# treangenlab/komb

Hardware: AMD Instinct MI355X
Metric: peeled edges/sec (k-truss) (higher is better)
Workload: dtype int32

## Files before the change

komb_amd/api.py:

```python
import ctypes
import os

import numpy as np

from . import _lib
from ._lib import KombOpts, KombStats, as_c, ptr


class KombError(RuntimeError):
    def __init__(self, code, msg):
        super().__init__(f"komb_accel error {code}: {msg}")
        self.code = code


def gen_hug_edges(nv, n_cliques, alpha=2.6, seed=42):
    lib = _lib.load()
    n_raw = lib.komb_gen_hug_edges(nv, n_cliques, alpha, seed, None)
    if n_raw < 0:
        raise ValueError("komb_gen_hug_edges: bad arguments")
    uv = np.empty((n_raw, 2), dtype=np.int64)
    got = lib.komb_gen_hug_edges(nv, n_cliques, alpha, seed, ptr(uv))
    assert got == n_raw
    return uv


FORWARD_ENV_OPTIONS = False
OPTION_NAMES = ("FINISH", "LOCAL_LIMIT", "LOCAL_ITEMS", "LOCAL_DENSITY", "LOCAL_DEFER_CHUNKS", "TAIL", "CORE_TAIL", "INDEX",
                "REC_CAP", "OWN_DENSE_CAP", "NO_OWN_DENSE", "NO_REC_SCRATCH", "NO_FIRST_QUEUE", "FULL_CAPS", "PREP_ROW_STAGE", "RETIRE_EVERY", "SHARD_ENGINE",
                "TRI_DEBUG", "POOL_DEBUG", "BUILD_DEBUG", "LOCAL_DEBUG", "TAIL_DEBUG", "COMP_SAMPLE", "COMM_SHORT", "COMM_HEAVY", "POISON")

SENTINEL_I32 = -0x5A5A5A5B


def _out_i32(n):
    return np.full(n, SENTINEL_I32, dtype=np.int32)


def _out_f64(n):
    return np.full(n, np.nan, dtype=np.float64)


class KombAccel:
    def __init__(self, device=0, verbosity=0, flags=0):
        self._lib = _lib.load()
        opts = KombOpts(device=device, verbosity=verbosity)
        opts.reserved[0] = flags
        self._ctx = self._lib.komb_create(ctypes.byref(opts))
        if not self._ctx:
            raise MemoryError("komb_create failed")
        self.device = device
        self.nv = -1
        self.ne = 0
        self._forwarded = {}

    def set_option(self, name, value):
        v = None if value is None else str(value).encode()
        self._check(self._lib.komb_set_option(self._ctx, name.encode(), v))

    def _sync_env_options(self):
        if not FORWARD_ENV_OPTIONS:
            return
        for name in OPTION_NAMES:
            v = os.environ.get("KOMB_" + name)
            if name == "INDEX" and os.environ.get("KOMB_TWO_PASS"):
                v = "two_pass"
            if name == "SHARD_ENGINE" and v is None:
                v = os.environ.get("KOMB_SHARD_PEEL")
            if self._forwarded.get(name) != v:
                self.set_option(name, v)
                self._forwarded[name] = v

    def close(self):
        if getattr(self, "_ctx", None):
            self._lib.komb_destroy(self._ctx)
            self._ctx = None

    def __del__(self):
        self.close()

    def __enter__(self):
        return self

    def __exit__(self, *a):
        self.close()

    def _check(self, rc):
        if rc != 0:
            raise KombError(rc, self._lib.komb_last_error(self._ctx).decode())

    def from_edges(self, nv, uv):
        uv = as_c(np.asarray(uv).reshape(-1, 2), np.int64)
        self._sync_env_options()
        self._check(self._lib.komb_graph_from_edges(self._ctx, nv, uv.shape[0], ptr(uv)))
        self._info()
        return self

    def from_csr(self, rowptr, col):
        rowptr = as_c(rowptr, np.int64)
        col = as_c(col, np.int32)
        self._sync_env_options()
        self._check(self._lib.komb_graph_from_csr(self._ctx, len(rowptr) - 1, ptr(rowptr), ptr(col)))
        self._info()
        return self

    def _info(self):
        nv, ne = ctypes.c_int64(), ctypes.c_int64()
        self._check(self._lib.komb_graph_info(self._ctx, ctypes.byref(nv), ctypes.byref(ne)))
        self.nv, self.ne = nv.value, ne.value

    def get_csr(self):
        rowptr = np.full(self.nv + 1, SENTINEL_I32, dtype=np.int64)
        col = _out_i32(2 * self.ne)
        self._check(self._lib.komb_graph_get_csr(self._ctx, ptr(rowptr), ptr(col)))
        return rowptr, col

    def core_run(self):
        self._sync_env_options()
        self._check(self._lib.komb_core_run(self._ctx))

    def set_shard_peel(self, on=True):
        self._check(self._lib.komb_set_shard_peel(self._ctx, 1 if on else 0))

    def core_fetch(self):
        deg = _out_i32(self.nv)
        core = _out_i32(self.nv)
        self._check(self._lib.komb_core_fetch(self._ctx, ptr(deg), ptr(core)))
        return deg, core

    def run_core(self):
        self.core_run()
        return self.core_fetch()

    def onion_run(self):
        self._sync_env_options()
        self._check(self._lib.komb_onion_run(self._ctx))

    def onion_fetch(self):
        layer = _out_i32(self.nv)
        core = _out_i32(self.nv)
        self._check(self._lib.komb_onion_fetch(self._ctx, ptr(layer), ptr(core)))
        return layer, core

    def run_onion(self):
        self.onion_run()
        return self.onion_fetch()

    def onion_info(self):
        n, k, ms = ctypes.c_int64(), ctypes.c_int32(), ctypes.c_double()
        self._check(self._lib.komb_onion_info(self._ctx, ctypes.byref(n), ctypes.byref(k), ctypes.byref(ms)))
        return {"n_layers": n.value, "max_coreness": k.value, "ms": ms.value}

    COMP_KINDS = {"core": _lib.KOMB_COMP_CORE, "truss": _lib.KOMB_COMP_TRUSS}

    def components_run(self, kind, k):
        self._sync_env_options()
        self._check(self._lib.komb_components_run(self._ctx, self.COMP_KINDS.get(kind, kind), k))

    def components_fetch(self):
        label = _out_i32(max(self.nv, 0))
        size = _out_i32(max(self.nv, 0))
        self._check(self._lib.komb_components_fetch(self._ctx, ptr(label), ptr(size)))
        return label, size

    def components_info(self):
        kind, k = ctypes.c_int32(), ctypes.c_int32()
        mem, comp, big, ms = ctypes.c_int64(), ctypes.c_int64(), ctypes.c_int64(), ctypes.c_double()
        self._check(self._lib.komb_components_info(self._ctx, ctypes.byref(kind), ctypes.byref(k), ctypes.byref(mem),
                                                   ctypes.byref(comp), ctypes.byref(big), ctypes.byref(ms)))
        return {"kind": kind.value, "k_used": k.value, "n_members": mem.value, "n_components": comp.value,
                "largest": big.value, "ms": ms.value}

    def run_components(self, kind="core", k=0):
        self.components_run(kind, k)
        return self.components_fetch()

    def truss_run(self, vmask=None):
        if vmask is not None:
            vmask = as_c(vmask, np.uint8)
            if len(vmask) != self.nv:
                raise ValueError("vmask must have nv entries")
        self._sync_env_options()
        self._check(self._lib.komb_truss_run(self._ctx, ptr(vmask)))

    def truss_run_slice(self, rank, world, vmask=None):
        if vmask is not None:
            vmask = as_c(vmask, np.uint8)
            if len(vmask) != self.nv:
                raise ValueError("vmask must have nv entries")
        self._sync_env_options()
        self._check(self._lib.komb_truss_run_slice(self._ctx, ptr(vmask), int(rank), int(world)))

    def truss_prepare(self):
        self._check(self._lib.komb_truss_prepare(self._ctx))

    def truss_unprepare(self):
        self._check(self._lib.komb_truss_unprepare(self._ctx))

    def graph_moments(self):
        self._check(self._lib.komb_graph_moments(self._ctx))

    def truss_fetch_into(self, eu=None, ev=None, tr=None):
        self._check(self._lib.komb_truss_fetch(self._ctx, ptr(eu) if eu is not None else None, ptr(ev) if ev is not None else None,
                                               ptr(tr) if tr is not None else None))

    def truss_fetch(self, with_support=False):
        n = ctypes.c_int64()
        self._check(self._lib.komb_truss_count(self._ctx, ctypes.byref(n)))
        eu = _out_i32(n.value)
        ev = _out_i32(n.value)
        tr = _out_i32(n.value)
        self._check(self._lib.komb_truss_fetch(self._ctx, ptr(eu), ptr(ev), ptr(tr)))
        if not with_support:
            return eu, ev, tr
        sup = _out_i32(n.value)
        self._check(self._lib.komb_truss_fetch_support(self._ctx, ptr(sup)))
        return eu, ev, tr, sup

    def run_truss(self, vmask=None, with_support=False):
        self.truss_run(vmask)
        return self.truss_fetch(with_support)

    def truss_communities_run(self, k=3):
        self._sync_env_options()
        self._check(self._lib.komb_truss_communities_run(self._ctx, k))

    def truss_communities_fetch(self):
        n = ctypes.c_int64()
        self._check(self._lib.komb_truss_count(self._ctx, ctypes.byref(n)))
        label = _out_i32(max(n.value, 0))
        size = _out_i32(max(n.value, 0))
        self._check(self._lib.komb_truss_communities_fetch(self._ctx, ptr(label), ptr(size)))
        return label, size

    def truss_communities_fetch_vertices(self):
        n_comm = _out_i32(max(self.nv, 0))
        self._check(self._lib.komb_truss_communities_fetch_vertices(self._ctx, ptr(n_comm)))
        return n_comm

    def truss_communities_info(self):
        k = ctypes.c_int32()
        mem, comm, big, multi, ms = ctypes.c_int64(), ctypes.c_int64(), ctypes.c_int64(), ctypes.c_int64(), ctypes.c_double()
        self._check(self._lib.komb_truss_communities_info(self._ctx, ctypes.byref(k), ctypes.byref(mem), ctypes.byref(comm),
                                                          ctypes.byref(big), ctypes.byref(multi), ctypes.byref(ms)))
        return {"k_used": k.value, "n_member_edges": mem.value, "n_communities": comm.value, "largest": big.value,
                "n_multi_vertices": multi.value, "ms": ms.value}

    def run_truss_communities(self, k=3):
        self.truss_communities_run(k)
        return self.truss_communities_fetch()

    def get_anomaly_score(self, degree, coreness):
        degree = as_c(degree, np.int32)
        coreness = as_c(coreness, np.int32)
        score = _out_f64(len(degree))
        self._sync_env_options()
        self._check(self._lib.komb_corea_scores(self._ctx, ptr(degree), ptr(coreness), len(degree), ptr(score)))
        return score

    def fractional_ranks(self, degree, coreness):
        degree = as_c(degree, np.int32)
        coreness = as_c(coreness, np.int32)
        rd = _out_f64(len(degree))
        rk = _out_f64(len(degree))
        self._sync_env_options()
        self._check(self._lib.komb_corea_ranks(self._ctx, ptr(degree), ptr(coreness), len(degree), ptr(rd), ptr(rk)))
        return rd, rk

    def densest_block(self, suspiciousness=None):
        n = int(self.nv)
        order = _out_i32(max(2 * n, 1))
        side = _out_i32(max(2 * n, 1))
        self._sync_env_options()
        nb = ctypes.c_int64(0)
        dens = ctypes.c_double(0.0)
        susp = None if suspiciousness is None else as_c(suspiciousness, np.float64)
        self._check(self._lib.komb_densest_block(self._ctx, ptr(susp), ptr(order), ptr(side), ctypes.byref(nb), ctypes.byref(dens)))
        return order[: 2 * n], side[: 2 * n], int(nb.value), float(dens.value)

    def stats(self):
        st = KombStats()
        self._check(self._lib.komb_get_stats(self._ctx, ctypes.byref(st)))
        return {name: getattr(st, name) for name, _ in KombStats._fields_}
```

komb_amd/csrc/common.h:

```cpp
#pragma once

#include <hip/hip_runtime.h>

#include <chrono>
#include <cstddef>
#include <cstdint>
#include <cstdio>
#include <cstdlib>
#include <cstring>
#include <map>
#include <string>
#include <vector>

#include "komb_accel.h"

#include <roctracer/roctx.h>

namespace komb {

struct Range {
    explicit Range(const char *name) { (void)roctxRangePushA(name); }
    ~Range() { (void)roctxRangePop(); }
    void next(const char *name) { (void)roctxRangePop(); (void)roctxRangePushA(name); }
    Range(const Range &) = delete;
    Range &operator=(const Range &) = delete;
};

constexpr int kBlock = 256;
constexpr int kWave = 64;
constexpr int32_t kAlive = 0x7FFFFFFF;
constexpr int32_t kAliveMin = 0x40000000;

struct PeelCtrl {
    int32_t  mode;
    int32_t  level;
    int32_t  round;
    int32_t  done;
    uint32_t cur_light;
    uint32_t cur_heavy;
    int32_t  cur_sel;
    uint32_t remaining;
    int32_t  n_levels;
    int32_t  n_rounds;
    int32_t  n_scans;
    int32_t  max_level;
    uint32_t live_count;
    int32_t  live_sel;
    int32_t  live_mode;
    int32_t  seq;
    uint32_t tail_l[2];
    uint32_t tail_h[2];
    int32_t  next_min;
    uint32_t live_tail;
    int32_t  last_retire;
    uint32_t tail_limit;
    uint32_t pad1[7];
    int32_t  max_retire_gap;
};
static_assert(offsetof(PeelCtrl, seq) == 60 && offsetof(PeelCtrl, tail_l) == 64, "PeelCtrl: the entry state is one 64-byte line");
static_assert(sizeof(PeelCtrl) == 128, "PeelCtrl layout");

struct LocalCtrl {
    int32_t  done;
    int32_t  iters;
    uint32_t spare[3];
    uint32_t bad;
    int32_t  max_val;
    uint32_t levels;
    uint32_t evals;
    uint32_t n_light, n_heavy;
    uint32_t n_giant;
    uint32_t n_chunk;
    uint32_t pad0;
    unsigned long long key_sum;
};
static_assert(sizeof(LocalCtrl) == 64, "LocalCtrl layout");

enum FinishMode : int { FIN_LOCAL = 0, FIN_LDS = 1, FIN_NONE = 2 };

struct Timer {
    hipEvent_t a = nullptr, b = nullptr;
    bool init() { return hipEventCreate(&a) == hipSuccess && hipEventCreate(&b) == hipSuccess; }
    void start(hipStream_t s) { (void)hipEventRecord(a, s); }
    double stop(hipStream_t s)
    {
        (void)hipEventRecord(b, s);
        (void)hipEventSynchronize(b);
        float ms = 0.f;
        (void)hipEventElapsedTime(&ms, a, b);
        return (double)ms;
    }
    void destroy() { if (a) (void)hipEventDestroy(a); if (b) (void)hipEventDestroy(b); a = b = nullptr; }
};

struct EventSet {
    std::vector<hipEvent_t> v;
    EventSet() = default;
    EventSet(const EventSet &) = delete;
    EventSet &operator=(const EventSet &) = delete;
    hipError_t make(hipEvent_t *out, unsigned flags = 0)
    {
        hipEvent_t e = nullptr;
        const hipError_t rc = flags ? hipEventCreateWithFlags(&e, flags) : hipEventCreate(&e);
        if (rc == hipSuccess) { v.push_back(e); *out = e; }
        return rc;
    }
    ~EventSet() { for (hipEvent_t e : v) if (e) (void)hipEventDestroy(e); }
};

}

struct Poison {
    bool on = false;
    uint32_t word = 0;
    hipStream_t stream = nullptr;
    hipError_t fill(void *p, size_t bytes) const
    {
        if (!on || !p || !bytes) return hipSuccess;
        const size_t words = bytes / 4, rest = bytes % 4;
        hipError_t e = hipSuccess;
        if (words) e = hipMemsetD32Async((hipDeviceptr_t)p, (int)word, words, stream);
        if (e == hipSuccess && rest) e = hipMemsetAsync((char *)p + 4 * words, (int)(word & 0xFFu), rest, stream);
        return e == hipSuccess ? hipStreamSynchronize(stream) : e;
    }
    hipError_t malloc(void **out, size_t bytes) const
    {
        void *q = nullptr;
        hipError_t e = hipMalloc(&q, bytes);
        if (e != hipSuccess) return e;
        e = fill(q, bytes);
        if (e != hipSuccess) { (void)hipFree(q); return e; }
        *out = q;
        return hipSuccess;
    }
};

struct DevPool {
    struct Block { void *p; size_t bytes; bool used; };
    std::vector<Block> blocks;
    size_t n_malloc = 0, n_trim = 0;
    double ms_malloc = 0.0;
    Poison poison;
    hipError_t get(void **out, size_t bytes)
    {
        if (bytes == 0) bytes = 16;
        int best = -1;
        for (int i = 0; i < (int)blocks.size(); ++i)
            if (!blocks[i].used && blocks[i].bytes >= bytes && blocks[i].bytes <= bytes + bytes / 4 + 4096 &&
                (best < 0 || blocks[i].bytes < blocks[best].bytes)) best = i;
        if (best >= 0) {
            if (poison.on) { const hipError_t e = poison.fill(blocks[best].p, blocks[best].bytes); if (e != hipSuccess) return e; }
            blocks[best].used = true; *out = blocks[best].p; return hipSuccess;
        }
        void *q = nullptr;
        ++n_malloc;
        const auto t0 = std::chrono::steady_clock::now();
        hipError_t e = hipMalloc(&q, bytes);
        ms_malloc += std::chrono::duration<double, std::milli>(std::chrono::steady_clock::now() - t0).count();
        if (e != hipSuccess) {
            ++n_trim;
            trim();
            e = hipMalloc(&q, bytes);
            if (e != hipSuccess) return e;
        }
        blocks.push_back({q, bytes, true});
        if (poison.on) { e = poison.fill(q, bytes); if (e != hipSuccess) { put(q); return e; } }
        *out = q;
        return hipSuccess;
    }
    void put(void *p)
    {
        if (!p) return;
        for (auto &b : blocks) if (b.p == p) { b.used = false; return; }
    }
    size_t unused_bytes() const
    {
        size_t t = 0;
        for (const auto &b : blocks) if (!b.used) t += b.bytes;
        return t;
    }
    void trim()
    {
        std::vector<Block> keep;
        for (auto &b : blocks) { if (b.used) keep.push_back(b); else (void)hipFree(b.p); }
        blocks.swap(keep);
    }
    void clear()
    {
        for (auto &b : blocks) (void)hipFree(b.p);
        blocks.clear();
    }
};

struct TrussPrep {
    bool valid = false;
    int64_t nv = 0, ne = 0;
    int32_t  *o2i = nullptr, *i2o = nullptr;
    uint32_t *orow = nullptr;
    int32_t  *ocol = nullptr, *osrc = nullptr;
    uint32_t *e2k = nullptr;
    uint4    *vline = nullptr;
    void     *wtasks = nullptr;
    int64_t   n_wtasks = 0;
    int64_t   own_bound = 0;
    double    ms = 0.0;
    double    ms_part[4] = {0, 0, 0, 0};
};

struct komb_ctx {
    komb_opts opts{};
    DevPool pool;
    std::string err;
    bool device_ok = false;
    int device = 0;
    hipStream_t stream = nullptr;
    bool own_stream = false;
    komb::Timer timer;
    std::map<std::string, std::string> options;

    int64_t nv = -1, ne = 0;
    uint32_t *d_o_rowptr = nullptr;
    int32_t  *d_o_col = nullptr;
    TrussPrep prep;

    int32_t *d_deg = nullptr;
    int32_t *d_core = nullptr;
    bool core_done = false;

    int32_t *d_onion_layer = nullptr;
    int32_t *d_onion_core = nullptr;
    int64_t onion_layers = 0;
    int32_t onion_max_core = 0;
    double onion_ms = 0.0;
    bool onion_done = false;

    int32_t *d_comp_label = nullptr;
    int32_t *d_comp_size = nullptr;
    int32_t comp_kind = 0, comp_k = 0;
    int64_t comp_members = 0, comp_count = 0, comp_largest = 0;
    double comp_ms = 0.0;
    bool comp_done = false;

    int32_t *d_comm_label = nullptr;
    int32_t *d_comm_size = nullptr;
    int32_t *d_comm_ncomm = nullptr;
    int32_t comm_k = 0;
    int64_t comm_members = 0, comm_count = 0, comm_largest = 0, comm_multi = 0;
    double comm_ms = 0.0, comm_ms_vertices = 0.0;
    bool comm_done = false, comm_v_ready = false;

    int64_t t_ne = -1;
    int32_t *d_t_eu = nullptr, *d_t_ev = nullptr, *d_t_truss = nullptr, *d_t_sup = nullptr;
    uint2 *d_t_slice = nullptr;
    uint32_t t_k_lo = 0, t_k_hi = 0;
    bool t_sup_ready = false;
    bool t_own_edges = false;
    int32_t *d_ceu = nullptr, *d_cev = nullptr;
    bool truss_done = false;
    int slice_rank = 0, slice_world = 1;
    bool shard_peel = false;
    struct { int64_t nv = -1, m = -1; unsigned long long own_cap = 0, rec_cap = 0; } cap_hint;

    komb::PeelCtrl *h_ctrl = nullptr;
    komb::LocalCtrl *h_local = nullptr;
    void *h_stage = nullptr;
    struct H2DStager *stager = nullptr;

    komb_stats stats{};
};

inline hipError_t dev_malloc(komb_ctx *ctx, void **out, size_t bytes) { return ctx->pool.poison.malloc(out, bytes); }

inline const char *ctx_opt(const komb_ctx *ctx, const char *name)
{
    const auto it = ctx->options.find(name);
    return it == ctx->options.end() ? nullptr : it->second.c_str();
}
inline bool ctx_flag(const komb_ctx *ctx, const char *name)
{
    const char *v = ctx_opt(ctx, name);
    return v && strcmp(v, "0") != 0;
}
namespace komb {
inline FinishMode finish_mode(const komb_ctx *ctx, FinishMode dflt)
{
    const char *e = ctx_opt(ctx, "FINISH");
    if (e && !strcmp(e, "local")) return FIN_LOCAL;
    if (e && !strcmp(e, "lds")) return FIN_LDS;
    if (e && !strcmp(e, "none")) return FIN_NONE;
    return dflt;
}
inline uint64_t local_item_limit(const komb_ctx *ctx, uint64_t dflt)
{
    if (const char *e = ctx_opt(ctx, "LOCAL_ITEMS")) return strtoull(e, nullptr, 10);
    return dflt;
}
inline uint32_t local_density_limit(const komb_ctx *ctx, uint32_t dflt)
{
    if (const char *e = ctx_opt(ctx, "LOCAL_DENSITY")) return (uint32_t)strtoul(e, nullptr, 10);
    return dflt;
}
inline uint32_t local_limit(const komb_ctx *ctx, uint64_t units, uint64_t divisor)
{
    uint64_t l = units / divisor;
    if (l < 4096) l = 4096;
    if (const char *e = ctx_opt(ctx, "LOCAL_LIMIT")) l = strtoull(e, nullptr, 10);
    if (l > units) l = units;
    return (uint32_t)l;
}
}

struct DevBufs {
    komb_ctx *ctx;
    std::vector<void *> owned;
    explicit DevBufs(komb_ctx *c) : ctx(c) {}
    DevBufs(const DevBufs &) = delete;
    DevBufs &operator=(const DevBufs &) = delete;
    template <class T> hipError_t alloc(T **out, size_t count)
    {
        void *q = nullptr;
        hipError_t e = ctx->pool.get(&q, (count ? count : 1) * sizeof(T));
        if (e == hipSuccess) { owned.push_back(q); *out = (T *)q; }
        return e;
    }
    void detach(void *q)
    {
        for (auto &p : owned) if (p == q) p = nullptr;
    }
    void release(void *q)
    {
        for (auto &p : owned) if (p == q && q) { ctx->pool.put(q); p = nullptr; }
    }
    ~DevBufs() { for (void *p : owned) if (p) ctx->pool.put(p); }
};

#define KOMB_FAIL(ctx, code, ...)                                   \
    do {                                                            \
        char _b[512];                                               \
        snprintf(_b, sizeof(_b), __VA_ARGS__);                      \
        (ctx)->err = _b;                                            \
        return (code);                                              \
    } while (0)

#define KOMB_HIP(ctx, call)                                                          \
    do {                                                                             \
        hipError_t _e = (call);                                                      \
        if (_e != hipSuccess) {                                                      \
            hipError_t _nomem = hipErrorOutOfMemory;                                 \
            KOMB_FAIL(ctx, _e == _nomem ? KOMB_ERR_NOMEM : KOMB_ERR_DEVICE,          \
                      "%s failed: %s (%s:%d)", #call, hipGetErrorString(_e),         \
                      __FILE__, __LINE__);                                           \
        }                                                                            \
    } while (0)

#define KOMB_TRY(expr)                         \
    do {                                       \
        int _s = (expr);                       \
        if (_s != KOMB_OK) return _s;          \
    } while (0)

constexpr size_t kStageBytes = 64 << 10;
inline hipError_t d2h(komb_ctx *ctx, void *dst, const void *src, size_t bytes)
{
    if (ctx->h_stage && bytes <= kStageBytes && dst != ctx->h_stage) {
        hipError_t e = hipMemcpyAsync(ctx->h_stage, src, bytes, hipMemcpyDeviceToHost, ctx->stream);
        if (e == hipSuccess) e = hipStreamSynchronize(ctx->stream);
        if (e == hipSuccess) memcpy(dst, ctx->h_stage, bytes);
        return e;
    }
    hipError_t e = hipMemcpyAsync(dst, src, bytes, hipMemcpyDeviceToHost, ctx->stream);
    return e == hipSuccess ? hipStreamSynchronize(ctx->stream) : e;
}

namespace komb {
int prim_sort_u64(komb_ctx *ctx, uint64_t *keys, uint64_t *tmp_keys, int64_t n, int end_bit, uint64_t **sorted);
int prim_unique_u64(komb_ctx *ctx, const uint64_t *in, uint64_t *out, int64_t n, int64_t *n_out);
int prim_exclusive_sum_u32(komb_ctx *ctx, const uint32_t *in, uint32_t *out, int64_t n);
int prim_exclusive_sum_u32_u64(komb_ctx *ctx, const uint32_t *in, unsigned long long *out, int64_t n);
int prim_sort_pairs_desc_i64(komb_ctx *ctx, int64_t *keys, int64_t *keys_tmp, uint32_t *vals, uint32_t *vals_tmp,
                             int64_t n, int end_bit, int64_t **sorted_keys, uint32_t **sorted_vals);

int prim_sort_pairs_u32_u64(komb_ctx *ctx, uint32_t *keys, uint32_t *keys_alt, unsigned long long *vals, unsigned long long *vals_alt,
                            int64_t n, int begin_bit, int end_bit, uint32_t **sorted_keys, unsigned long long **sorted_vals);
int prim_sort_pairs_u32_u32(komb_ctx *ctx, uint32_t *keys, uint32_t *keys_alt, uint32_t *vals, uint32_t *vals_alt,
                            int64_t n, int end_bit, uint32_t **sorted_keys, uint32_t **sorted_vals);
int prim_sort_pairs_u64_u32(komb_ctx *ctx, uint64_t *keys, uint64_t *keys_alt, uint32_t *vals, uint32_t *vals_alt,
                            int64_t n, int end_bit, uint64_t **sorted_keys, uint32_t **sorted_vals);

int core_run(komb_ctx *ctx, int rank = 0, int world = 1, komb_allreduce_fn fn = nullptr, void *user = nullptr, bool sharded = false);
int onion_run(komb_ctx *ctx);
int components_run(komb_ctx *ctx, int32_t kind, int32_t k);
int communities_run(komb_ctx *ctx, int32_t k);
int communities_vertices(komb_ctx *ctx);
void communities_drop(komb_ctx *ctx);
int truss_run(komb_ctx *ctx, const uint8_t *vmask_host, int rank, int world, komb_allreduce_fn fn, void *user);
int merge_run(komb_ctx *ctx, const double *susp_host, int32_t *order, int32_t *side, int64_t *n_block, double *max_density);
int corea_ranks(komb_ctx *ctx, const int32_t *deg, const int32_t *core, int64_t n, double *rank_deg, double *rank_key);
int graph_from_edges(komb_ctx *ctx, int64_t nv, int64_t n_raw, const int64_t *uv);
int graph_from_csr(komb_ctx *ctx, int64_t nv, const int64_t *rowptr, const int32_t *col);
void graph_free(komb_ctx *ctx);
void stager_free(komb_ctx *ctx);
hipError_t staged_copy(komb_ctx *ctx, void *dst, const void *src, size_t bytes, bool to_device);
void warm_up(komb_ctx *ctx);
int prep_build(komb_ctx *ctx, const uint32_t *rowptr, const int32_t *col, int64_t nv, int64_t ns, TrussPrep *out);
void prep_free(komb_ctx *ctx, TrussPrep *p);
int prep_ensure(komb_ctx *ctx);
int prep_sources(komb_ctx *ctx, TrussPrep *p);
int graph_moments(komb_ctx *ctx, int64_t out[5]);
struct InducedCsr { int64_t nv = 0, ns = 0; uint32_t *rowptr = nullptr; int32_t *col = nullptr; int32_t *vold = nullptr; };
int induce_csr(komb_ctx *ctx, const uint8_t *vmask_host, InducedCsr *out);
void induced_free(komb_ctx *ctx, InducedCsr *g);
int edge_list(komb_ctx *ctx, const uint32_t *rowptr, const int32_t *col, int64_t nv, const int32_t *vold, int32_t *eu, int32_t *ev);
int truss_edges_canonical(komb_ctx *ctx);
void truss_free(komb_ctx *ctx);
int truss_support_canonical(komb_ctx *ctx);
void peel_ctrl_pre(hipStream_t s, uint32_t *d_grp_done);
void peel_collect_ctrl(hipStream_t s, PeelCtrl *d_collect, const PeelCtrl *d_from);
void peel_ctrl_init(hipStream_t s, PeelCtrl *d_ctrl, uint32_t *d_grp_done, uint32_t units, uint32_t tail_limit = 0);
int peel_grid(int64_t units);

template <typename F>
int drive_peel(komb_ctx *ctx, PeelCtrl *d_ctrl, int64_t units, F &&launch, int *launches_out)
{
#ifndef KOMB_PEEL_BATCH
#define KOMB_PEEL_BATCH 24
#endif
#ifndef KOMB_PEEL_BATCH_SHORT
#define KOMB_PEEL_BATCH_SHORT 6
#endif
    constexpr int kBatch = KOMB_PEEL_BATCH, kBatchShort = KOMB_PEEL_BATCH_SHORT, kShortBatches = 6;
    PeelCtrl first;
    KOMB_HIP(ctx, d2h(ctx, &first, d_ctrl, sizeof(PeelCtrl)));
    int32_t next = first.seq;
#ifdef KOMB_DEBUG_SWITCHES
    if (const char *tr = getenv("KOMB_PEEL_TRACE")) {
        FILE *f = fopen(tr, "a");
        hipEvent_t a = nullptr, b = nullptr;
        if (hipEventCreate(&a) != hipSuccess || hipEventCreate(&b) != hipSuccess) {
            if (f) fclose(f);
            if (a) (void)hipEventDestroy(a);
            KOMB_FAIL(ctx, KOMB_ERR_DEVICE, "peel trace: hipEventCreate failed");
        }
        int launches = 0;
        if (f) fprintf(f, "# peel units=%lld\n", (long long)units);
        for (int64_t i = 0; i < 4 * units + 4096; ++i) {
            PeelCtrl before;
            if (d2h(ctx, &before, d_ctrl, sizeof(PeelCtrl)) != hipSuccess) break;
            if (before.done) break;
            (void)hipEventRecord(a, ctx->stream);
            launch(before.seq); ++launches;
            (void)hipEventRecord(b, ctx->stream);
            (void)hipEventSynchronize(b);
            float ms = 0.f;
            (void)hipEventElapsedTime(&ms, a, b);
            if (f) fprintf(f, "%d %d %d %u %u %d %u %u %.1f\n", before.mode, before.level, before.round, before.cur_light,
                           before.cur_heavy, before.live_mode, before.live_count, before.remaining, ms * 1000.f);
        }
        if (f) fclose(f);
        (void)hipEventDestroy(a); (void)hipEventDestroy(b);
        if (launches_out) *launches_out = launches;
        KOMB_HIP(ctx, d2h(ctx, &ctx->h_ctrl[0], d_ctrl, sizeof(PeelCtrl)));
        return KOMB_OK;
    }
#endif
    EventSet evs;
    hipEvent_t ev[2] = {nullptr, nullptr};
    KOMB_HIP(ctx, evs.make(&ev[0], hipEventDisableTiming));
    KOMB_HIP(ctx, evs.make(&ev[1], hipEventDisableTiming));
    const int64_t max_batches = (4 * units + 4096) / kBatch + 16 + kShortBatches;
    int launches = 0, slot = 0, status = KOMB_OK;
    bool have_prev = false, finished = false, stuck = false;
    int32_t seen_seq = first.seq - 1;
    for (int64_t batch = 0; batch < max_batches && !finished; ++batch) {
        const int nb = (batch >= 1 && batch <= kShortBatches) ? kBatchShort : kBatch;
        for (int i = 0; i < nb; ++i) { launch(next); ++next; ++launches; }
        if (hipMemcpyAsync(&ctx->h_ctrl[slot], d_ctrl, sizeof(PeelCtrl), hipMemcpyDeviceToHost, ctx->stream) != hipSuccess ||
            hipEventRecord(ev[slot], ctx->stream) != hipSuccess) { status = KOMB_ERR_DEVICE; break; }
        if (have_prev) {
            if (hipEventSynchronize(ev[slot ^ 1]) != hipSuccess) { status = KOMB_ERR_DEVICE; break; }
            const PeelCtrl &h = ctx->h_ctrl[slot ^ 1];
            if (h.done) finished = true;
            else if (h.seq == seen_seq) { stuck = true; finished = true; }
            seen_seq = h.seq;
        }
        have_prev = true;
        slot ^= 1;
    }
    hipError_t e = hipStreamSynchronize(ctx->stream);
    if (launches_out) *launches_out = launches;
    if (status != KOMB_OK || e != hipSuccess)
        KOMB_FAIL(ctx, KOMB_ERR_DEVICE, "peel driver: HIP failure (%s)", hipGetErrorString(e));
    if (d2h(ctx, &ctx->h_ctrl[0], d_ctrl, sizeof(PeelCtrl)) != hipSuccess)
        KOMB_FAIL(ctx, KOMB_ERR_DEVICE, "peel driver: control block readback failed");
    if (!ctx->h_ctrl[0].done)
        KOMB_FAIL(ctx, KOMB_ERR_DEVICE, "peel driver: %s (level %d, remaining %u, launch %d of state %d)",
                  stuck ? "the launches make no progress" : "launch budget exhausted before completion",
                  ctx->h_ctrl[0].level, ctx->h_ctrl[0].remaining, (int)next, (int)ctx->h_ctrl[0].seq);
    return KOMB_OK;
}
}
```

komb_amd/csrc/ktruss.hip:

```cpp
#include "peel_dev.h"
#include "truss_tail.h"
#include "local_dev.h"
#include "shard_dev.h"

#include <algorithm>
#include <cstdlib>
#include <cstring>

#include "truss_line.h"
#include "truss_tri.h"
#include "truss_wedge.h"
#include "truss_index.h"
#include "truss_gather.h"

namespace komb {

namespace {

struct TrussProblem {
    static constexpr bool kChain = false;
    static constexpr bool kSingleStep = false;
    uint32_t units;
    const uint2 *off2;
    const int2 *inc;
    int32_t *sup;
    int32_t *stamp;
    uint8_t *st8;
    static constexpr int32_t kRetireEvery = komb::kRetireEvery;
    int32_t retire_every;
#ifdef KOMB_DEBUG_SWITCHES
    int ablate;
#endif

    __device__ __forceinline__ void retire(const CtrlView &cv, uint32_t block, uint32_t nblocks) const
    {
        const uint32_t n16 = (units + 15u) / 16u;
        uint4 *v = reinterpret_cast<uint4 *>(st8);
        for (uint32_t i = block * (uint32_t)kPeelBlock + threadIdx.x; i < n16; i += nblocks * (uint32_t)kPeelBlock) {
            uint4 q = v[i];
            uint32_t *w = &q.x;
            bool changed = false;
#pragma unroll
            for (int k = 0; k < 4; ++k) {
                uint32_t out = w[k];
#pragma unroll
                for (int b = 0; b < 4; ++b) {
                    const uint32_t c = (w[k] >> (8 * b)) & 0xFFu;
                    if (c > ST_GONE && state_rel(c, cv.round) == REL_GONE) out = (out & ~(0xFFu << (8 * b))) | ((uint32_t)ST_GONE << (8 * b));
                }
                changed |= out != w[k];
                w[k] = out;
            }
            if (changed) v[i] = q;
        }
    }

    __device__ __forceinline__ const int32_t *scan_marker() const { return stamp; }
    __device__ __forceinline__ const uint8_t *scan_state() const { return st8; }
    __device__ __forceinline__ const int32_t *scan_key() const { return sup; }
    __device__ __forceinline__ void mark_scanned(uint32_t e, const CtrlView &cv) const { stamp[e] = cv.round; st8[e] = state_of_round(cv.round); }
    __device__ __forceinline__ void slice(uint32_t e, uint32_t &b, uint32_t &len) const
    {
        const uint2 o = off2[e];
        b = o.x;
        len = o.y;
    }
    struct Loaded { int32_t me, x, y; uint32_t cx, cy; };
    __device__ __forceinline__ Loaded item_load(int32_t me, uint32_t pos, const CtrlView &) const
    {
        Loaded ld;
#ifdef KOMB_DEBUG_SWITCHES
        if (ablate & 6) {
            int2 p = make_int2((int)(((uint32_t)me * 2654435761u) % units), (int)(((uint32_t)me * 40503u + pos) % units));
            if (!(ablate & 4)) { const unsigned long long pq = __builtin_nontemporal_load(reinterpret_cast<const unsigned long long *>(inc) + pos); p = make_int2((int)(uint32_t)pq, (int)(uint32_t)(pq >> 32)); }
            ld.me = me; ld.x = p.x; ld.y = p.y;
            ld.cx = (ablate & 2) ? 0u : st8[p.x]; ld.cy = (ablate & 2) ? 0u : st8[p.y];
            return ld;
        }
#endif
        const unsigned long long pq = __builtin_nontemporal_load(reinterpret_cast<const unsigned long long *>(inc) + pos);
        const int2 p = make_int2((int)(uint32_t)pq, (int)(uint32_t)(pq >> 32));
        ld.me = me; ld.x = p.x; ld.y = p.y;
        ld.cx = st8[p.x]; ld.cy = st8[p.y];
        return ld;
    }
    __device__ __forceinline__ void item_apply(const Loaded &ld, const CtrlView &cv, int32_t &t0, int32_t &t1, uint32_t &c0, uint32_t &c1) const
    {
        const int32_t r = cv.round, L = cv.level;
        const int rx = state_rel(ld.cx, r), ry = state_rel(ld.cy, r);
        if (rx == REL_GONE || ry == REL_GONE) return;
        const bool xin = (rx == REL_NOW), yin = (ry == REL_NOW);
        bool decx = !xin && (!yin || ld.me < ld.y);
        bool decy = !yin && (!xin || ld.me < ld.x);
#ifdef KOMB_DEBUG_SWITCHES
        if (ablate & 1) { decx = false; decy = false; }
#endif
        if (decx && atomicSub(&sup[ld.x], 1) == L + 1) {
            c0 = ld.cx == ST_ALIVE_HEAVY ? marker_chunks(stamp[ld.x]) : 0u;
            stamp[ld.x] = r + 1; st8[ld.x] = state_of_round(r + 1); t0 = ld.x;
        }
        if (decy && atomicSub(&sup[ld.y], 1) == L + 1) {
            c1 = ld.cy == ST_ALIVE_HEAVY ? marker_chunks(stamp[ld.y]) : 0u;
            stamp[ld.y] = r + 1; st8[ld.y] = state_of_round(r + 1); t1 = ld.y;
        }
    }
};

struct ShardTruss {
    static constexpr bool kChain = false;
    static constexpr bool kSingleStep = true;
    uint32_t units;
    const uint2 *off2;
    const int2 *inc;
    int32_t *sup;
    int32_t *stamp;
    uint32_t lo, hi;

    __device__ __forceinline__ const int32_t *scan_marker() const { return stamp; }
    __device__ __forceinline__ const int32_t *scan_key() const { return sup; }
    __device__ __forceinline__ void mark_scanned(uint32_t e, const CtrlView &cv) const { stamp[e] = cv.round; }
    __device__ __forceinline__ void slice(uint32_t e, uint32_t &b, uint32_t &len) const
    {
        const uint2 o = off2[e];
        b = o.x;
        len = o.y;
    }
    __device__ __forceinline__ bool mine(int32_t e) const { return (uint32_t)e - lo < hi - lo; }
    struct Loaded { int32_t me, x, y, sx, sy; };
    __device__ __forceinline__ Loaded item_load(int32_t me, uint32_t pos, const CtrlView &) const
    {
        Loaded ld;
        const int2 p = inc[pos];
        ld.me = me; ld.x = p.x; ld.y = p.y;
        ld.sx = stamp[p.x]; ld.sy = stamp[p.y];
        return ld;
    }
    __device__ __forceinline__ void item_apply(const Loaded &ld, const CtrlView &cv, int32_t &t0, int32_t &t1, uint32_t &, uint32_t &) const
    {
        const int32_t r = cv.round, L = cv.level;
        if (ld.sx < r || ld.sy < r) return;
        const bool xin = (ld.sx == r), yin = (ld.sy == r);
        const bool decx = !xin && (!yin || ld.me < ld.y) && mine(ld.x);
        const bool decy = !yin && (!xin || ld.me < ld.x) && mine(ld.y);
        if (decx && atomicSub(&sup[ld.x], 1) == L + 1) { stamp[ld.x] = r + 1; t0 = ld.x; }
        if (decy && atomicSub(&sup[ld.y], 1) == L + 1) { stamp[ld.y] = r + 1; t1 = ld.y; }
    }
};

struct TrussCollect {
    static constexpr bool kChain = false;
    static constexpr bool kSingleStep = false;
    uint32_t units;
    const uint2 *off2;
    const int2 *inc;
    const int32_t *stamp;
    const int32_t *num;
    const uint32_t *coff;
    uint32_t *cur;
    uint2 *cpair;

    __device__ __forceinline__ const int32_t *scan_marker() const { return stamp; }
    __device__ __forceinline__ const int32_t *scan_key() const { return nullptr; }
    __device__ __forceinline__ void mark_scanned(uint32_t, const CtrlView &) const {}
    __device__ __forceinline__ void slice(uint32_t e, uint32_t &b, uint32_t &len) const
    {
        const uint2 o = off2[e];
        b = o.x;
        len = o.y;
    }
    struct Loaded { int32_t me, x, y, sx, sy; };
    __device__ __forceinline__ Loaded item_load(int32_t me, uint32_t pos, const CtrlView &) const
    {
        Loaded ld;
        const int2 p = inc[pos];
        ld.me = me; ld.x = p.x; ld.y = p.y;
        ld.sx = stamp[p.x]; ld.sy = stamp[p.y];
        return ld;
    }
    __device__ __forceinline__ void item_apply(const Loaded &ld, const CtrlView &, int32_t &, int32_t &, uint32_t &, uint32_t &) const
    {
        if (!marker_alive(ld.sx) || !marker_alive(ld.sy)) return;
        const uint32_t id = (uint32_t)num[ld.me];
        const uint32_t b0 = coff[id], k = local_slot(id, cur);
        if (k < coff[id + 1] - b0) cpair[b0 + k] = make_uint2((uint32_t)num[ld.x], (uint32_t)num[ld.y]);
    }
};

constexpr uint64_t kTrussLocalItems = 32ull << 20;
constexpr uint32_t kTrussLocalDensity = 160;
struct TrussLocal {
    static constexpr int kU = 8;
#ifndef KOMB_TRUSS_GROUPS
#define KOMB_TRUSS_GROUPS 8
#endif
    static constexpr int kGroups = KOMB_TRUSS_GROUPS;
    static constexpr int kN = 2;
    const uint2 *cpair;
    __device__ __forceinline__ void ids(uint32_t pos, uint32_t (&id)[2]) const
    {
        const uint2 p = cpair[pos];
        id[0] = p.x; id[1] = p.y;
    }
};

}

void truss_free(komb_ctx *ctx)
{
    communities_drop(ctx);
    if (ctx->t_own_edges) { ctx->pool.put(ctx->d_t_eu); ctx->pool.put(ctx->d_t_ev); }
    ctx->pool.put(ctx->d_t_truss);
    ctx->pool.put(ctx->d_t_sup);
    ctx->pool.put(ctx->d_t_slice);
    ctx->d_t_eu = ctx->d_t_ev = ctx->d_t_truss = ctx->d_t_sup = nullptr;
    ctx->d_t_slice = nullptr;
    ctx->t_sup_ready = false;
    ctx->t_own_edges = false;
    ctx->t_ne = -1; ctx->truss_done = false;
}

int truss_edges_canonical(komb_ctx *ctx)
{
    if (ctx->t_own_edges || ctx->t_ne <= 0) return KOMB_OK;
    if (!ctx->d_ceu) {
        int32_t *eu = nullptr, *ev = nullptr;
        hipError_t e = ctx->pool.get((void **)&eu, (size_t)ctx->ne * sizeof(int32_t));
        if (e == hipSuccess) e = ctx->pool.get((void **)&ev, (size_t)ctx->ne * sizeof(int32_t));
        const int rc = e == hipSuccess ? edge_list(ctx, ctx->d_o_rowptr, ctx->d_o_col, ctx->nv, nullptr, eu, ev) : KOMB_ERR_NOMEM;
        if (rc != KOMB_OK) {
            ctx->pool.put(eu); ctx->pool.put(ev);
            if (e != hipSuccess) KOMB_FAIL(ctx, KOMB_ERR_NOMEM, "komb_truss_fetch: no memory for the canonical edge list (%s)", hipGetErrorString(e));
            return rc;
        }
        ctx->d_ceu = eu; ctx->d_cev = ev;
    }
    ctx->d_t_eu = ctx->d_ceu; ctx->d_t_ev = ctx->d_cev;
    return KOMB_OK;
}

int truss_support_canonical(komb_ctx *ctx)
{
    if (ctx->t_sup_ready) return KOMB_OK;
    if (!ctx->truss_done || !ctx->d_t_slice || !ctx->prep.valid || ctx->prep.ne != ctx->t_ne)
        KOMB_FAIL(ctx, KOMB_ERR_STATE, "komb_truss_fetch_support: no k-truss result to take the supports from");
    hipStream_t s = ctx->stream;
    const int64_t m = ctx->t_ne;
    KOMB_HIP(ctx, ctx->pool.get((void **)&ctx->d_t_sup, (size_t)m * sizeof(int32_t)));
#ifndef KOMB_TEST_SKIP_SLICE_ZERO
    if (ctx->t_k_lo) KOMB_HIP(ctx, hipMemsetAsync(ctx->d_t_sup, 0, (size_t)ctx->t_k_lo * sizeof(int32_t), s));
    if (ctx->t_k_hi < (uint32_t)m) KOMB_HIP(ctx, hipMemsetAsync(ctx->d_t_sup + ctx->t_k_hi, 0, ((size_t)m - ctx->t_k_hi) * sizeof(int32_t), s));
#endif
    k_scatter_len<<<grid_for(m), kBlock, 0, s>>>(ctx->d_t_slice, ctx->prep.e2k, m, ctx->t_k_lo, ctx->t_k_hi, ctx->d_t_sup);
    KOMB_HIP(ctx, hipStreamSynchronize(s));
    ctx->t_sup_ready = true;
    return KOMB_OK;
}

int truss_run(komb_ctx *ctx, const uint8_t *vmask_host, int rank, int world, komb_allreduce_fn fn, void *user)
{
    if (world < 1 || rank < 0 || rank >= world || (world > 1 && !fn))
        KOMB_FAIL(ctx, KOMB_ERR_ARG, "komb_truss_run_sharded: bad rank %d / world %d / callback", rank, world);
    if (ctx->nv < 0) KOMB_FAIL(ctx, KOMB_ERR_STATE, "komb_truss_run: no graph loaded");
    truss_free(ctx);
    hipStream_t s = ctx->stream;
    komb_stats &st = ctx->stats;
    st.triangles = 0; st.truss_levels = st.truss_subrounds = st.truss_launches = 0;
    st.max_trussness = 0; st.ms_support = st.ms_peel = st.ms_orient = st.ms_tri_count = st.ms_tri_fill = st.ms_gather = st.ms_allreduce = st.ms_compact = 0.0;
    st.truss_scans = 0; st.ms_prepare = 0.0; st.truss_prepared = 0; st.ms_prep_vertex = st.ms_prep_edges = st.ms_prep_rows = 0.0;
    auto empty_result = [&]() -> int {
        KOMB_HIP(ctx, ctx->pool.get((void **)&ctx->d_t_eu, 4)); KOMB_HIP(ctx, ctx->pool.get((void **)&ctx->d_t_ev, 4));
        KOMB_HIP(ctx, ctx->pool.get((void **)&ctx->d_t_truss, 4)); KOMB_HIP(ctx, ctx->pool.get((void **)&ctx->d_t_sup, 4));
        ctx->t_own_edges = true; ctx->t_ne = 0; ctx->truss_done = true; ctx->t_sup_ready = true;
        return KOMB_OK;
    };
    if (ctx->nv == 0 || ctx->ne == 0) return empty_result();
    Range r_all("komb_truss_run");
    DevBufs bufs(ctx);

    Range phase("truss: preparation");
    InducedCsr sub;
    TrussPrep sub_prep;
    struct SubGuard { komb_ctx *c; InducedCsr *g; TrussPrep *p; ~SubGuard() { prep_free(c, p); induced_free(c, g); } } sub_guard{ctx, &sub, &sub_prep};
    TrussPrep *tp = &ctx->prep;
    if (vmask_host) {
        ctx->timer.start(s);
        KOMB_TRY(induce_csr(ctx, vmask_host, &sub));
        st.ms_orient = ctx->timer.stop(s);
        if (sub.ns == 0) return empty_result();
        KOMB_TRY(prep_build(ctx, sub.rowptr, sub.col, sub.nv, sub.ns, &sub_prep));
        st.ms_prepare = sub_prep.ms; st.truss_prepared = 1;
        st.ms_prep_vertex = sub_prep.ms_part[0]; st.ms_prep_edges = sub_prep.ms_part[1]; st.ms_prep_rows = sub_prep.ms_part[2];
        tp = &sub_prep;
    } else if (!ctx->prep.valid) {
        KOMB_TRY(prep_ensure(ctx));
        st.ms_prepare = ctx->prep.ms; st.truss_prepared = 1;
        st.ms_prep_vertex = ctx->prep.ms_part[0]; st.ms_prep_edges = ctx->prep.ms_part[1]; st.ms_prep_rows = ctx->prep.ms_part[2];
    }
    const int64_t nv = tp->nv;
    const int64_t m = tp->ne;
    const uint32_t *d_orow = tp->orow;
    const int32_t *d_ocol = tp->ocol;
    const uint4 *d_line = tp->vline;
    const uint2 *d_wtasks = (const uint2 *)tp->wtasks;
    const int64_t n_wtasks = tp->n_wtasks;
    const int gw = grid_for(n_wtasks, kTriWaves);
    phase.next("truss: triangles + incidence index");

    const int ge = grid_for(m);
    const int tri_tv = (int)std::max<int64_t>(1, std::min<int64_t>(kTriV, nv / (256 * KOMB_TRI_EU * kTriWaves * 4)));
    const int64_t ntasks = (nv + tri_tv - 1) / tri_tv;
    const int gt = grid_for(ntasks, kTriWaves);
    uint32_t *d_own = nullptr, *d_other = nullptr, *d_cnt = nullptr, *d_off = nullptr;
    uint2 *d_off2 = nullptr;
    KOMB_HIP(ctx, bufs.alloc(&d_own, 2 * ((size_t)m + 1)));
    d_other = d_own + ((size_t)m + 1);
    KOMB_HIP(ctx, bufs.alloc(&d_cnt, (size_t)m + 1));
    KOMB_HIP(ctx, bufs.alloc(&d_off2, (size_t)m + 4));
    unsigned long long *d_mom = nullptr;
    KOMB_HIP(ctx, bufs.alloc(&d_mom, 12));
    KOMB_HIP(ctx, hipMemsetAsync(d_mom, 0, 12 * sizeof(unsigned long long), s));
    st.ms_allreduce = 0.0;

    const FinishMode fin = finish_mode(ctx, FIN_LOCAL);
    if (fin == FIN_LDS) KOMB_TRY(prep_sources(ctx, tp));
    const int32_t *d_osrc = tp->osrc;
    uint32_t tail_limit = 0;
    if (fin == FIN_LDS) {
        tail_limit = kTailEdges;
        if (const char *tl = ctx_opt(ctx, "TAIL")) tail_limit = (uint32_t)strtoul(tl, nullptr, 10);
        if (tail_limit > kTailMaxEdges) tail_limit = kTailMaxEdges;
    } else if (fin == FIN_LOCAL) tail_limit = local_limit(ctx, (uint64_t)m, 32);
    const bool whole_peel_finish = tail_limit && (uint64_t)m <= tail_limit;
    const bool shard_peel_on = (ctx->shard_peel && world > 1) || ctx_flag(ctx, "SHARD_ENGINE");
    enum { IDX_STREAM = 0, IDX_TWO_PASS = 2 };
    int layout = IDX_STREAM;
    if (const char *ix = ctx_opt(ctx, "INDEX")) {
        if (!strcmp(ix, "two_pass")) layout = IDX_TWO_PASS;
        else if (strcmp(ix, "stream")) KOMB_FAIL(ctx, KOMB_ERR_ARG, "option INDEX=%s: expected stream or two_pass", ix);
    }
    int2 *d_owndense = nullptr;
    unsigned long long *d_ownoff = nullptr, *d_dcur = nullptr;
    uint32_t *d_cnt_ref = nullptr;
    uint32_t *d_toff = nullptr;
    uint32_t *d_grp = nullptr;
    int32_t *d_light0 = nullptr;
    uint32_t *d_bintot = nullptr;
    uint32_t *d_reckey = nullptr;
    int2 *d_recval = nullptr;
    const BinGeom geom = bin_geom(m);
    const int64_t n_bins = (int64_t)geom.nb;
    const TriStream no_stream{nullptr, nullptr, nullptr, 0ull, 0u, 0u, 0};
#ifdef KOMB_DEBUG_SWITCHES
    const int ablate = getenv("KOMB_TRI_ABLATE") ? atoi(getenv("KOMB_TRI_ABLATE")) : 0;
#else
    const int ablate = 0;
#endif
    st.ms_sort = 0.0; st.tri_records = 0; st.ms_compact = 0.0; st.ms_tri_count = 0.0; st.ms_tri_fill = 0.0; st.stream_retries = 0;
    st.index_layout = layout;
    auto zero_counts = [&]() -> hipError_t { return hipMemsetAsync(d_own, 0, 2 * ((size_t)m + 1) * sizeof(uint32_t), s); };
    if (!(world == 1 && layout == IDX_STREAM)) KOMB_HIP(ctx, zero_counts());
    bool have_counts = false;
    if (world > 1) {
        const int64_t task_lo = n_wtasks * rank / world, task_hi = n_wtasks * (rank + 1) / world;
        ctx->timer.start(s);
        k_wedges<TRI_COUNT><<<gw, kBlock, 0, s>>>(d_orow, d_ocol, d_line, d_wtasks, task_lo, task_hi, d_own, d_other, nullptr, nullptr, 0ull, nullptr, no_stream, nullptr, ablate);
        st.ms_tri_count = ctx->timer.stop(s);
        k_sum_counts<<<ge, kBlock, 0, s>>>(d_own, d_other, nullptr, m + 1, d_cnt, d_mom + 5);
        ctx->timer.start(s);
        KOMB_HIP(ctx, hipStreamSynchronize(s));
        if (fn(user, d_cnt, (int64_t)m + 1) != 0)
            KOMB_FAIL(ctx, KOMB_ERR_DEVICE, "komb_truss_run_sharded: all-reduce callback failed");
        st.ms_allreduce = ctx->timer.stop(s);
        KOMB_HIP(ctx, hipMemsetAsync(d_mom + 5, 0, sizeof(unsigned long long), s));
        k_total_u32<<<ge, kBlock, 0, s>>>(d_cnt, m + 1, d_mom + 5);
        have_counts = true;
        if (layout != IDX_TWO_PASS) {
            KOMB_HIP(ctx, bufs.alloc(&d_cnt_ref, (size_t)m + 1));
            KOMB_HIP(ctx, hipMemcpyAsync(d_cnt_ref, d_cnt, ((size_t)m + 1) * sizeof(uint32_t), hipMemcpyDeviceToDevice, s));
            KOMB_HIP(ctx, zero_counts());
        }
    }

    if (layout == IDX_STREAM) {
        const unsigned long long bound = (unsigned long long)tp->own_bound;
        const int gws = std::min(gw, 256 * KOMB_WEDGE_EU);
        const unsigned long long slack = (unsigned long long)gws * kTriWaves * kRecChunk + kRecChunk;
        const unsigned long long own_slack = (unsigned long long)gws * kTriWaves * kOwnChunk + kOwnChunk;
        const unsigned long long t_bound = bound / 2;
        const unsigned long long own_full = bound + bound / 8 + own_slack, rec_full = 3 * t_bound + (3 * t_bound) / 14 + slack;
        unsigned long long own_cap = std::min(own_full, 4ull * (unsigned long long)m + own_slack);
        unsigned long long rec_cap = std::min(rec_full, 2ull * (unsigned long long)m + slack);
        bool fixed_caps = false;
        if (const char *oc = ctx_opt(ctx, "OWN_DENSE_CAP")) { own_cap = strtoull(oc, nullptr, 10) + 1; rec_cap = rec_full; fixed_caps = true; }
        if (ctx_flag(ctx, "NO_OWN_DENSE")) { own_cap = 1; rec_cap = rec_full; fixed_caps = true; }
        if (const char *rc = ctx_opt(ctx, "REC_CAP")) { rec_cap = strtoull(rc, nullptr, 10) + 1; fixed_caps = true; }
        if (ctx_flag(ctx, "FULL_CAPS")) { own_cap = own_full; rec_cap = rec_full; }
        if (!fixed_caps && ctx->cap_hint.nv == nv && ctx->cap_hint.m == m) {
            own_cap = std::min(own_full, std::max(own_cap, ctx->cap_hint.own_cap));
            rec_cap = std::min(rec_full, std::max(rec_cap, ctx->cap_hint.rec_cap));
        }
        const uint32_t sentinel = geom.sentinel_base();
        uint32_t *d_key = nullptr; int2 *d_val = nullptr;
        unsigned long long n_claimed = 0;
        bool ok = false;
        st.ms_tri_fill = 0.0;
        for (int attempt = 0; attempt < 2; ++attempt) {
            size_t free_b = 0, total_b = 0;
            (void)hipMemGetInfo(&free_b, &total_b);
            const unsigned long long budget = (unsigned long long)((free_b + ctx->pool.unused_bytes()) * 0.7);
            if (own_cap * sizeof(int2) > budget / 2) own_cap = budget / 2 / sizeof(int2);
            if (rec_cap * 12ull > budget / 2) rec_cap = budget / 2 / 12ull;
            if (rec_cap > 0xFFFFFFF0ull) rec_cap = 0xFFFFFFF0ull;
            ok = bufs.alloc(&d_key, (size_t)rec_cap) == hipSuccess && bufs.alloc(&d_val, (size_t)rec_cap) == hipSuccess &&
                 bufs.alloc(&d_owndense, (size_t)own_cap) == hipSuccess &&
                 (d_ownoff || bufs.alloc(&d_ownoff, (size_t)m + 1) == hipSuccess) && (d_dcur || bufs.alloc(&d_dcur, 4) == hipSuccess);
            uint2 *d_scratch = nullptr;
            if (ok && !ctx_flag(ctx, "NO_REC_SCRATCH") && bufs.alloc(&d_scratch, (size_t)gws * kTriWaves * kScratchRec) != hipSuccess) { (void)hipGetLastError(); d_scratch = nullptr; }
            if (!ok) { (void)hipGetLastError(); break; }
            KOMB_HIP(ctx, hipMemsetAsync(d_dcur, 0, 4 * sizeof(unsigned long long), s));
            const TriStream ts{d_key, d_val, d_dcur + 2, rec_cap, sentinel, geom.nb - 1u, kChunkBits};
            ctx->timer.start(s);
            k_wedges<TRI_SINGLE><<<gws, kBlock, 0, s>>>(d_orow, d_ocol, d_line, d_wtasks, 0, n_wtasks, d_own, d_other, d_owndense, d_dcur, own_cap, d_ownoff, ts, d_scratch, ablate);
            st.ms_tri_fill += ctx->timer.stop(s);
            unsigned long long dc[4] = {0, 0, 0, 0};
            KOMB_HIP(ctx, d2h(ctx, dc, d_dcur, sizeof(dc)));
            n_claimed = dc[2];
            bufs.release(d_scratch);
            if (ctx_flag(ctx, "TRI_DEBUG"))
                fprintf(stderr, "komb triangles: stream build (attempt %d): %llu record positions claimed of %llu, dense own-role region %llu entries claimed of %llu, %llu task ranges overflowed their record buffer\n",
                        attempt, dc[2], rec_cap, dc[0], own_cap, dc[1]);
            if (n_claimed <= rec_cap) {
                if (!fixed_caps) { ctx->cap_hint.nv = nv; ctx->cap_hint.m = m; ctx->cap_hint.own_cap = own_cap; ctx->cap_hint.rec_cap = rec_cap; }
                break;
            }
            ok = false;
            if (attempt == 1 || fixed_caps) break;
            bufs.release(d_key); bufs.release(d_val); bufs.release(d_owndense);
            d_key = nullptr; d_val = nullptr; d_owndense = nullptr;
            own_cap = std::min(own_full, std::max(own_cap, dc[0] + own_slack));
            rec_cap = std::min(rec_full, n_claimed + slack);
            st.stream_retries += 1;
        }
        uint32_t *d_skey = nullptr;
        if (ok) {
            uint32_t *d_key2 = nullptr; unsigned long long *d_val2 = nullptr;
            ok = bufs.alloc(&d_key2, (size_t)n_claimed + 1) == hipSuccess && bufs.alloc(&d_val2, (size_t)n_claimed + 1) == hipSuccess;
            if (ok) {
                ctx->timer.start(s);
                unsigned long long *sv = nullptr;
                if (geom.nb_bits > 0) KOMB_TRY(prim_sort_pairs_u32_u64(ctx, d_key, d_key2, (unsigned long long *)d_val, d_val2, (int64_t)n_claimed, kChunkBits, kChunkBits + geom.nb_bits, &d_skey, &sv));
                else { d_skey = d_key; sv = (unsigned long long *)d_val; }
                st.ms_sort = ctx->timer.stop(s);
                d_recval = (int2 *)sv;
                if (d_skey == d_key) { bufs.release(d_key2); bufs.release(d_val2); } else { bufs.release(d_key); bufs.release(d_val); }
                d_reckey = d_skey;
                KOMB_HIP(ctx, bufs.alloc(&d_toff, (size_t)n_bins + 2));
                KOMB_HIP(ctx, bufs.alloc(&d_bintot, (size_t)n_bins + 2));
                KOMB_HIP(ctx, bufs.alloc(&d_grp, (size_t)kInitOff + 4));
                if (!whole_peel_finish && !shard_peel_on && !ctx_flag(ctx, "NO_FIRST_QUEUE")) KOMB_HIP(ctx, bufs.alloc(&d_light0, (size_t)m));
                ctx->timer.start(s);
                peel_ctrl_pre(s, d_grp);
                KOMB_HIP(ctx, hipMemsetAsync(d_mom + 5, 0, sizeof(unsigned long long), s));
                k_bin_offsets<<<grid_for(n_bins + 1), kBlock, 0, s>>>(d_skey, (int64_t)n_claimed, geom, d_toff);
                k_bin_count<<<grid_for(n_bins, 1, 256 * 8), kBlock, 0, s>>>(d_skey, d_toff, geom, d_own, m, d_cnt, d_bintot, d_mom + 5, (int32_t *)(d_grp + kInitOff + 1));
                st.ms_compact = ctx->timer.stop(s);
                st.tri_records = (int64_t)n_claimed;
            } else (void)hipGetLastError();
        }
        if (!ok) {
            bufs.release(d_key); bufs.release(d_val); bufs.release(d_owndense); bufs.release(d_ownoff); bufs.release(d_dcur);
            bufs.release(d_grp); bufs.release(d_light0); d_grp = nullptr; d_light0 = nullptr;
            d_owndense = nullptr; d_ownoff = nullptr; d_dcur = nullptr;
            KOMB_HIP(ctx, zero_counts());
            KOMB_HIP(ctx, hipMemsetAsync(d_mom + 5, 0, sizeof(unsigned long long), s));
            st.ms_tri_fill = 0.0;
            layout = IDX_TWO_PASS;
        }
    }
    if (layout != IDX_TWO_PASS && d_cnt_ref) {
        k_count_mismatch<<<ge, kBlock, 0, s>>>(d_cnt, d_cnt_ref, m + 1, d_mom + 8);
    }
    if (layout == IDX_TWO_PASS) {
        if (d_cnt_ref) {
            KOMB_HIP(ctx, hipMemcpyAsync(d_cnt, d_cnt_ref, ((size_t)m + 1) * sizeof(uint32_t), hipMemcpyDeviceToDevice, s));
            KOMB_HIP(ctx, hipMemsetAsync(d_mom + 5, 0, sizeof(unsigned long long), s));
            k_total_u32<<<ge, kBlock, 0, s>>>(d_cnt, m + 1, d_mom + 5);
        } else if (!have_counts) {
            ctx->timer.start(s);
            k_triangles<TRI_COUNT><<<gt, kBlock, 0, s>>>(d_orow, d_ocol, nv, 0, ntasks, d_own, d_other, nullptr, nullptr, ablate, tri_tv);
            st.ms_tri_count = ctx->timer.stop(s);
            k_sum_counts<<<ge, kBlock, 0, s>>>(d_own, d_other, nullptr, m + 1, d_cnt, d_mom + 5);
        }
    }
    st.index_layout = layout;
    {
        unsigned long long mom[9];
        KOMB_HIP(ctx, d2h(ctx, mom, d_mom, sizeof(mom)));
        st.triangles = (int64_t)(mom[5] / 3);
        bufs.release(d_mom);
        if (mom[8] != 0)
            KOMB_FAIL(ctx, KOMB_ERR_DEVICE, "komb_truss_run_sharded: %llu edges whose all-reduced support differs from the support of the index build", mom[8]);
        if (mom[5] > 0xFFFFFFF0ull)
            KOMB_FAIL(ctx, KOMB_ERR_LIMIT, "graph has %llu triangles; the incidence index is limited to 2^32-16 entries (3 per triangle)",
                      mom[5] / 3);
    }
    bufs.release(d_cnt_ref);
    uint32_t total = 0;
    const uint32_t sum_supports = (uint32_t)st.triangles * 3u;
    int2 *d_inc = nullptr;
    int32_t *d_sup = nullptr, *d_stamp = nullptr, *d_truss = nullptr;
    uint8_t *d_st8 = nullptr;
    bool peel_inited = false;
    if (layout == IDX_STREAM) {
        KOMB_TRY(prim_exclusive_sum_u32(ctx, d_bintot, d_bintot, n_bins + 1));
        total = sum_supports;
        KOMB_HIP(ctx, bufs.alloc(&d_inc, (size_t)total));
        KOMB_HIP(ctx, bufs.alloc(&d_sup, (size_t)m));
        KOMB_HIP(ctx, bufs.alloc(&d_stamp, (size_t)m));
        KOMB_HIP(ctx, bufs.alloc(&d_st8, (size_t)m + 16));
        KOMB_HIP(ctx, bufs.alloc(&d_truss, (size_t)m));
        ctx->timer.start(s);
        k_bin_finish<<<grid_for(n_bins, 1, 256 * kFinPerCu), kFinBlock, 0, s>>>(d_reckey, d_recval, d_toff, geom, d_own, d_cnt, d_bintot, d_owndense, d_ownoff, d_inc, m,
                                                                      d_off2, d_sup, d_stamp, d_st8, d_grp + kInitOff, d_light0);
        st.ms_compact += ctx->timer.stop(s);
        peel_inited = true;
        bufs.release(d_toff); bufs.release(d_bintot); bufs.release((void *)d_recval); bufs.release(d_reckey);
        bufs.release(d_owndense); bufs.release(d_ownoff); bufs.release(d_dcur);
    } else {
        KOMB_HIP(ctx, bufs.alloc(&d_off, (size_t)m + 1));
        KOMB_TRY(prim_exclusive_sum_u32(ctx, d_cnt, d_off, m + 1));
        KOMB_HIP(ctx, d2h(ctx, &total, d_off + m, sizeof(uint32_t)));
        KOMB_HIP(ctx, bufs.alloc(&d_inc, (size_t)total));
        ctx->timer.start(s);
        KOMB_HIP(ctx, zero_counts());
        k_back_cursors<<<ge, kBlock, 0, s>>>(d_off, m, d_other);
        k_triangles<TRI_SINGLE><<<gt, kBlock, 0, s>>>(d_orow, d_ocol, nv, 0, ntasks, d_own, d_other, d_off, d_inc, ablate, tri_tv);
        st.ms_tri_fill = ctx->timer.stop(s);
    }
    st.ms_support = st.ms_tri_count + st.ms_tri_fill + st.ms_sort + st.ms_compact;
    bufs.release(d_cnt); bufs.release(d_own);

    phase.next("truss: peel");
    PeelCtrl *d_ctrl = nullptr;
    PeelQueues Q{nullptr, {nullptr, nullptr}, {nullptr, nullptr}, {nullptr, nullptr}, 0};
    const size_t heavy_cap = (size_t)total / 32 + 64;
    if (!peel_inited) {
        KOMB_HIP(ctx, bufs.alloc(&d_sup, (size_t)m));
        KOMB_HIP(ctx, bufs.alloc(&d_stamp, (size_t)m));
        KOMB_HIP(ctx, bufs.alloc(&d_st8, (size_t)m + 16));
        KOMB_HIP(ctx, bufs.alloc(&d_truss, (size_t)m));
        KOMB_HIP(ctx, bufs.alloc(&d_grp, (size_t)kInitOff + 4));
    }
    for (int i = 0; i < 2; ++i) {
        if (i == 0 && d_light0) Q.light[0] = d_light0;
        else KOMB_HIP(ctx, bufs.alloc(&Q.light[i], (size_t)m));
        KOMB_HIP(ctx, bufs.alloc(&Q.heavy[i], heavy_cap));
        KOMB_HIP(ctx, bufs.alloc(&Q.live[i], (size_t)m / 2 + 64));
    }
    KOMB_HIP(ctx, bufs.alloc(&d_ctrl, 1));
    KOMB_HIP(ctx, bufs.alloc(&Q.code, (size_t)m));
    KOMB_HIP(ctx, bufs.alloc(&Q.rlevel, (size_t)m + 2));
    KOMB_HIP(ctx, hipMemsetAsync(Q.rlevel, 0, 2 * sizeof(int32_t), s));
    int32_t retire_every = kRetireEvery;
    if (const char *e = ctx_opt(ctx, "RETIRE_EVERY")) retire_every = std::max(1, std::min((int)kRetireEvery, atoi(e)));
#ifdef KOMB_DEBUG_SWITCHES
    TrussProblem P{(uint32_t)m, d_off2, d_inc, d_sup, d_stamp, d_st8, retire_every, getenv("KOMB_PEEL_ABLATE") ? atoi(getenv("KOMB_PEEL_ABLATE")) : 0};
#else
    TrussProblem P{(uint32_t)m, d_off2, d_inc, d_sup, d_stamp, d_st8, retire_every};
#endif
    TailBufs T{};
    if (fin == FIN_LDS && tail_limit) {
        KOMB_HIP(ctx, bufs.alloc(&T.vmap, (size_t)nv));
        KOMB_HIP(ctx, bufs.alloc(&T.cnt, 64));
        KOMB_HIP(ctx, bufs.alloc(&T.vlist, (size_t)kTailMaxV));
        KOMB_HIP(ctx, bufs.alloc(&T.rows, (size_t)kTailMaxV * kTailRowWords));
        KOMB_HIP(ctx, bufs.alloc(&T.pair, (size_t)tail_limit));
        KOMB_HIP(ctx, bufs.alloc(&T.sup, (size_t)tail_limit));
        KOMB_HIP(ctx, bufs.alloc(&T.gid, (size_t)tail_limit));
        KOMB_HIP(ctx, bufs.alloc(&T.gid_by_rank, (size_t)tail_limit));
        KOMB_HIP(ctx, bufs.alloc(&T.pair_by_rank, (size_t)tail_limit));
        KOMB_HIP(ctx, bufs.alloc(&T.truss_by_rank, (size_t)tail_limit));
        KOMB_HIP(ctx, bufs.alloc(&T.spill[0], (size_t)tail_limit));
        KOMB_HIP(ctx, bufs.alloc(&T.spill[1], (size_t)tail_limit));
        T.max_edges = tail_limit;
    }
    auto run_tail = [&](const int32_t *list, uint32_t n_in) -> int {
        KOMB_HIP(ctx, hipMemsetAsync(T.vmap, 0, (size_t)nv * sizeof(int32_t), s));
        KOMB_HIP(ctx, hipMemsetAsync(T.cnt, 0, 64 * sizeof(uint32_t), s));
        KOMB_HIP(ctx, hipMemsetAsync(T.rows, 0, (size_t)kTailMaxV * kTailRowWords * sizeof(unsigned long long), s));
        const int g = grid_for(n_in, kBlock, 256);
        const bool dbg = ctx_flag(ctx, "TAIL_DEBUG");
        hipEvent_t ev[3] = {nullptr, nullptr, nullptr};
        for (auto &e : ev) (void)hipEventCreate(&e);
        (void)hipEventRecord(ev[0], s);
        k_tail_mark<<<g, kBlock, 0, s>>>(list, n_in, d_sup, d_stamp, d_osrc, d_ocol, T);
        k_tail_number<<<1, kTailMaxV, 0, s>>>(T);
        k_tail_rows<<<g, kBlock, 0, s>>>(list, n_in, d_sup, d_stamp, d_osrc, d_ocol, T);
        (void)hipEventRecord(ev[1], s);
        k_truss_tail<<<1, 1024, 0, s>>>(d_ctrl, T, d_truss);
        (void)hipEventRecord(ev[2], s);
        KOMB_HIP(ctx, d2h(ctx, &ctx->h_ctrl[0], d_ctrl, sizeof(PeelCtrl)));
        ++st.truss_tail_runs;
        float m0 = 0, m1 = 0, m2 = 0;
        (void)hipEventElapsedTime(&m0, ctx->timer.a, ev[0]); (void)hipEventElapsedTime(&m1, ev[0], ev[1]); (void)hipEventElapsedTime(&m2, ev[1], ev[2]);
        for (auto &e : ev) (void)hipEventDestroy(e);
        st.ms_tail += (double)m1 + (double)m2;
        if (dbg) {
            uint32_t h[16];
            KOMB_HIP(ctx, d2h(ctx, h, T.cnt, sizeof(h)));
            fprintf(stderr, "komb tail: %u vertices, %u edges, %s; general engine before it %.1f us, setup %.1f us, tail kernel %.1f us\n",
                    h[0], h[1], ctx->h_ctrl[0].done == 1 ? "done" : "refused", m0 * 1000.f, m1 * 1000.f, m2 * 1000.f);
#ifdef KOMB_TAIL_TIMERS
            fprintf(stderr, "komb tail: us in kernel: load %.1f ranks %.1f supports %.1f scan %.1f mark %.1f triangles %.1f retire %.1f results %.1f\n",
                    h[14] / 100.0, h[15] / 100.0, h[8] / 100.0, h[9] / 100.0, h[10] / 100.0, h[11] / 100.0, h[12] / 100.0, h[13] / 100.0);
#endif
        }
        return KOMB_OK;
    };
    const int gp = peel_grid(m);
    auto run_local = [&]() -> int {
        const PeelCtrl hc = ctx->h_ctrl[0];
        EventSet evs;
        hipEvent_t ev[2] = {nullptr, nullptr};
        for (auto &e : ev) KOMB_HIP(ctx, evs.make(&e));
        (void)hipEventRecord(ev[0], s);
        LocalStats ls;
        const int lrc = local_finish(ctx, bufs, hc, d_ctrl, (uint32_t)m, d_stamp, d_sup, Q.live[hc.live_sel],
            (uint32_t)kWave * TrussLocal::kU, sizeof(uint2), local_item_limit(ctx, kTrussLocalItems), local_density_limit(ctx, kTrussLocalDensity), true, 2, d_truss,
            [&](const LocalGraph &lg, const int32_t *num, void *items, PeelCtrl *d_cctrl, int32_t launch) {
                TrussCollect C{(uint32_t)m, d_off2, d_inc, d_stamp, num, lg.off, lg.cur, (uint2 *)items};
                PeelQueues Qc = Q;
                Qc.rlevel = nullptr;
                k_peel_step<TrussCollect><<<gp, kPeelBlock, 0, s>>>(d_cctrl, d_grp, Qc, C, launch);
            },
            [&](const LocalGraph &lg, void *items, uint64_t total_items, LocalCtrl *d_lctrl, uint32_t *d_cnt, int *nl) -> int {
                return local_fixpoint(ctx, d_lctrl, d_cnt, lg, TrussLocal{(const uint2 *)items}, total_items, nl);
            },
            &ls, [](const LocalGraph &) {});
        (void)hipEventRecord(ev[1], s);
        (void)hipEventSynchronize(ev[1]);
        float ms = 0.f;
        (void)hipEventElapsedTime(&ms, ev[0], ev[1]);
        KOMB_TRY(lrc);
        if (ls.refused) { ctx->h_ctrl[0].done = 0; ctx->h_ctrl[0].tail_limit = ls.new_limit; return KOMB_OK; }
        st.truss_local_units = (int32_t)ls.units; st.truss_local_sweeps = ls.sweeps; st.truss_local_items = (int64_t)ls.items;
        st.ms_truss_local = (double)ms;
        PeelCtrl fin_c = hc;
        fin_c.done = 1; fin_c.remaining = 0;
        fin_c.n_levels += (int32_t)ls.levels;
        fin_c.max_level = ls.max_val > fin_c.max_level ? ls.max_val : fin_c.max_level;
        ctx->h_ctrl[0] = fin_c;
        return KOMB_OK;
    };
    ctx->timer.start(s);
    if (!peel_inited) {
        peel_ctrl_pre(s, d_grp);
        k_peel_init<<<grid_for(m, kBlock, 1024), kBlock, 0, s>>>(m, d_off, d_off2, d_sup, d_stamp, d_st8, d_grp + kInitOff);
    }
    peel_ctrl_init(s, d_ctrl, d_grp, (uint32_t)m, tail_limit);
    int launches = 0, rc = KOMB_OK;
    st.truss_tail_runs = 0; st.ms_tail = 0.0;
    st.truss_local_units = 0; st.truss_local_sweeps = 0; st.truss_local_items = 0; st.ms_truss_local = 0.0;
    st.shard_exchanges = 0; st.ms_exchange = 0.0; st.exchange_words = 0;
    if (shard_peel_on) {
        uint32_t iw[2] = {0u, 0u};
        KOMB_HIP(ctx, d2h(ctx, iw, d_grp + kInitOff, sizeof(iw)));
        ShardTruss SP{(uint32_t)m, d_off2, d_inc, d_sup, d_stamp, 0u, 0u};
        shard_bounds((uint64_t)m, rank, world, &SP.lo, &SP.hi);
        ShardStats ss;
        rc = shard_peel(ctx, bufs, SP, d_sup, (uint32_t)m, iw[0], (int32_t)iw[1], rank, world, fn, user, Q, d_ctrl,
                        [&](int32_t launch) { k_peel_step<ShardTruss><<<gp, kPeelBlock, 0, s>>>(d_ctrl, d_grp, Q, SP, launch); },
                        fin == FIN_LOCAL ? tail_limit : 0u, [&]() -> int { return run_local(); }, &ss);
        st.shard_exchanges = (int32_t)ss.exchanges; st.ms_exchange = ss.ms_exchange; st.exchange_words = ss.words;
        launches = ss.launches;
        PeelCtrl fc{};
        fc.done = rc == KOMB_OK ? 1 : 2; fc.n_levels = ss.levels; fc.n_rounds = ss.rounds; fc.n_scans = ss.scans; fc.max_level = ss.max_level;
        ctx->h_ctrl[0] = fc;
    } else if (whole_peel_finish) {
        rc = d2h(ctx, &ctx->h_ctrl[0], d_ctrl, sizeof(PeelCtrl)) == hipSuccess ? KOMB_OK : KOMB_ERR_DEVICE;
        if (rc == KOMB_OK && !ctx->h_ctrl[0].done) rc = (fin == FIN_LOCAL) ? run_local() : run_tail(nullptr, (uint32_t)m);
    } else {
        ctx->h_ctrl[0].done = 0;
    }
    for (int guard = 0; rc == KOMB_OK && ctx->h_ctrl[0].done != 1 && ctx->h_ctrl[0].done != 2 && guard < 64; ++guard) {
        if (ctx->h_ctrl[0].done == 3) {
            const PeelCtrl &c = ctx->h_ctrl[0];
            if (fin == FIN_LOCAL) rc = run_local();
            else rc = c.live_mode ? run_tail(Q.live[c.live_sel], c.live_count) : run_tail(nullptr, (uint32_t)m);
            continue;
        }
        int batch = 0;
        rc = drive_peel(ctx, d_ctrl, m, [&](int32_t launch) {
            k_peel_step<TrussProblem><<<gp, kPeelBlock, 0, s>>>(d_ctrl, d_grp, Q, P, launch);
        }, &batch);
        launches += batch;
    }
    st.ms_peel = ctx->timer.stop(s);
    KOMB_TRY(rc);
#ifdef KOMB_STEP_TIMERS
    {
        const PeelCtrl &c = ctx->h_ctrl[0];
        const double n = c.pad1[6] ? (double)c.pad1[6] : 1.0;
        fprintf(stderr, "komb step timers (block 0, %u small multi-workgroup PROCESS steps), us per step: ctrl %.2f queue+slice %.2f items %.2f flush %.2f barrier %.2f ticket %.2f\n",
                c.pad1[6], c.pad1[0] / n / 100.0, c.pad1[1] / n / 100.0, c.pad1[2] / n / 100.0, c.pad1[3] / n / 100.0, c.pad1[4] / n / 100.0, c.pad1[5] / n / 100.0);
    }
#endif
    if (ctx->h_ctrl[0].done != 1) KOMB_FAIL(ctx, KOMB_ERR_DEVICE, "k-truss peel ended in an inconsistent state");
    if (ctx->h_ctrl[0].max_retire_gap > retire_every)
        KOMB_FAIL(ctx, KOMB_ERR_DEVICE, "k-truss peel: %d sub-rounds passed without a RETIRE step (period %d): edge state codes may have wrapped",
                  ctx->h_ctrl[0].max_retire_gap, retire_every);
    st.engine_flags = (layout == IDX_TWO_PASS ? KOMB_ENGINE_TWO_PASS : 0) | (shard_peel_on ? KOMB_ENGINE_SHARD_PEEL : 0) |
                      (st.truss_local_units ? KOMB_ENGINE_LOCAL_FINISH : 0) | (st.truss_tail_runs ? KOMB_ENGINE_LDS_TAIL : 0);
    st.truss_levels = ctx->h_ctrl[0].n_levels;
    st.truss_subrounds = ctx->h_ctrl[0].n_rounds;
    st.truss_launches = launches;
    st.truss_scans = ctx->h_ctrl[0].n_scans;
    st.max_trussness = ctx->h_ctrl[0].max_level + 2;
    for (int i = 0; i < 2; ++i) { bufs.release(Q.light[i]); bufs.release(Q.heavy[i]); bufs.release(Q.live[i]); }
    bufs.release(Q.code);
    bufs.release(d_sup); bufs.release(d_inc);

    phase.next("truss: canonical gather");
    ctx->timer.start(s);
    KOMB_HIP(ctx, ctx->pool.get((void **)&ctx->d_t_truss, (size_t)m * sizeof(int32_t)));
    uint32_t k_lo = 0, k_hi = (uint32_t)m;
    if (!vmask_host) {
        ctx->d_t_eu = ctx->d_ceu; ctx->d_t_ev = ctx->d_cev;
        ctx->t_own_edges = false;
        if (ctx->slice_world > 1) {
            shard_bounds((uint64_t)m, ctx->slice_rank, ctx->slice_world, &k_lo, &k_hi);
#ifndef KOMB_TEST_SKIP_SLICE_ZERO
            if (k_lo) KOMB_HIP(ctx, hipMemsetAsync(ctx->d_t_truss, 0, (size_t)k_lo * sizeof(int32_t), s));
            if (k_hi < (uint32_t)m) KOMB_HIP(ctx, hipMemsetAsync(ctx->d_t_truss + k_hi, 0, ((size_t)m - k_hi) * sizeof(int32_t), s));
#endif
        }
    } else {
        ctx->t_own_edges = true;
        KOMB_HIP(ctx, ctx->pool.get((void **)&ctx->d_t_eu, (size_t)m * sizeof(int32_t)));
        KOMB_HIP(ctx, ctx->pool.get((void **)&ctx->d_t_ev, (size_t)m * sizeof(int32_t)));
        KOMB_TRY(edge_list(ctx, sub.rowptr, sub.col, sub.nv, sub.vold, ctx->d_t_eu, ctx->d_t_ev));
    }
    ctx->t_k_lo = k_lo; ctx->t_k_hi = k_hi;
    k_truss_results<<<grid_for(m), kBlock, 0, s>>>(d_stamp, Q.rlevel, d_truss, tp->e2k, m, k_lo, k_hi, ctx->d_t_truss);
    ctx->d_t_slice = d_off2;
    bufs.detach(d_off2);
    ctx->t_sup_ready = false;
    if (vmask_host) {
        ctx->t_ne = m;
        KOMB_HIP(ctx, ctx->pool.get((void **)&ctx->d_t_sup, (size_t)m * sizeof(int32_t)));
        k_scatter_len<<<grid_for(m), kBlock, 0, s>>>(ctx->d_t_slice, tp->e2k, m, 0u, (uint32_t)m, ctx->d_t_sup);
        ctx->t_sup_ready = true;
    }
    st.ms_gather = ctx->timer.stop(s);
    if (ctx_flag(ctx, "POOL_DEBUG")) {
        size_t held = 0;
        for (const auto &b : ctx->pool.blocks) held += b.bytes;
        fprintf(stderr, "komb pool: %zu blocks, %.2f GB held, %zu hipMalloc calls so far (%.1f ms inside them), %zu trims\n", ctx->pool.blocks.size(), held / 1e9, ctx->pool.n_malloc, ctx->pool.ms_malloc, ctx->pool.n_trim);
    }
    if (vmask_host) KOMB_HIP(ctx, hipStreamSynchronize(s));
    ctx->t_ne = m;
    ctx->truss_done = true;
    return KOMB_OK;
}

}
```

komb_amd/csrc/truss_index.h:

```cpp
#pragma once

#include "peel_dev.h"

namespace komb {

namespace {

constexpr int kBinBits = 11;
constexpr uint32_t kBinEdges = 1u << kBinBits;
#ifndef KOMB_CHUNK_BITS
#define KOMB_CHUNK_BITS 6
#endif
constexpr int kChunkBits = KOMB_CHUNK_BITS;
constexpr uint32_t kChunkMask = (1u << kChunkBits) - 1u;
struct BinGeom {
    int nb_bits;
    uint32_t nb;
    __host__ __device__ uint32_t bin_of(uint32_t e) const { return (e >> kChunkBits) & (nb - 1u); }
    __host__ __device__ uint32_t local_of(uint32_t e) const { return ((e >> (kChunkBits + nb_bits)) << kChunkBits) | (e & kChunkMask); }
    __host__ __device__ uint64_t edge_of(uint32_t b, uint32_t i) const
    {
        return ((((uint64_t)(i >> kChunkBits) << nb_bits) | b) << kChunkBits) | (i & kChunkMask);
    }
    __host__ __device__ uint32_t sentinel_base() const { return (uint32_t)(((uint64_t)kBinEdges >> kChunkBits) << (kChunkBits + nb_bits)); }
};
inline BinGeom bin_geom(int64_t m)
{
    BinGeom g{0, 1u};
    while (((int64_t)g.nb << kBinBits) < m) { ++g.nb_bits; g.nb <<= 1; }
    return g;
}

__global__ __launch_bounds__(kBlock) void k_bin_offsets(const uint32_t *__restrict__ key, int64_t n, BinGeom g, uint32_t *__restrict__ boff)
{
    for (int64_t b = (int64_t)blockIdx.x * kBlock + threadIdx.x; b <= (int64_t)g.nb; b += (int64_t)gridDim.x * kBlock) {
        int64_t lo = 0, hi = n;
        while (lo < hi) {
            const int64_t mid = lo + ((hi - lo) >> 1);
            if ((int64_t)g.bin_of(key[mid]) < b) lo = mid + 1; else hi = mid;
        }
        boff[b] = (uint32_t)lo;
    }
}

__global__ __launch_bounds__(kBlock) void k_count_mismatch(const uint32_t *__restrict__ a, const uint32_t *__restrict__ b, int64_t n,
                                                           unsigned long long *__restrict__ bad)
{
    unsigned long long t = 0;
    for (int64_t e = (int64_t)blockIdx.x * kBlock + threadIdx.x; e < n; e += (int64_t)gridDim.x * kBlock) t += a[e] != b[e] ? 1ull : 0ull;
    block_add_u64(t, bad);
}

__global__ __launch_bounds__(kBlock) void k_bin_count(const uint32_t *__restrict__ key, const uint32_t *__restrict__ boff, BinGeom g,
                                                      const uint32_t *__restrict__ own, int64_t m, uint32_t *__restrict__ sum,
                                                      uint32_t *__restrict__ bin_total, unsigned long long *__restrict__ total,
                                                      int32_t *__restrict__ min_pos)
{
    __shared__ uint32_t sh_cnt[kBinEdges];
    __shared__ uint32_t sh_part[kBlock / kWave];
    unsigned long long t = 0;
    int32_t lmin = 0x7FFFFFFF;
    for (uint32_t b = blockIdx.x; b < g.nb; b += gridDim.x) {
        for (uint32_t i = threadIdx.x; i < kBinEdges; i += kBlock) sh_cnt[i] = 0u;
        __syncthreads();
        const uint32_t r0 = boff[b], r1 = boff[b + 1];
        for (uint32_t r = r0 + threadIdx.x; r < r1; r += kBlock) {
            const uint32_t k = key[r];
            if ((int64_t)k < m) atomicAdd(&sh_cnt[g.local_of(k)], 1u);
        }
        __syncthreads();
        uint32_t tb = 0;
        for (uint32_t i = threadIdx.x; i < kBinEdges; i += kBlock) {
            const uint64_t e = g.edge_of(b, i);
            if (e >= (uint64_t)m) continue;
            const uint32_t c = own[e] + sh_cnt[i];
            sum[e] = c;
            tb += c;
            if (c) lmin = min(lmin, (int32_t)c);
        }
        tb = wave_sum(tb);
        if (lane_id() == 0) sh_part[threadIdx.x >> 6] = tb;
        __syncthreads();
        if (threadIdx.x == 0) {
            uint32_t all = 0;
            for (int i = 0; i < kBlock / kWave; ++i) all += sh_part[i];
            bin_total[b] = all;
            t += all;
        }
        __syncthreads();
    }
    if (blockIdx.x == 0 && threadIdx.x == 0) { sum[m] = 0u; bin_total[g.nb] = 0u; }
    if (threadIdx.x == 0 && t) atomicAdd(total, t);
    lmin = wave_min(lmin);
    if (lane_id() == 0 && lmin != 0x7FFFFFFF) atomicMin(min_pos, lmin);
}

constexpr int kFinBlock = 512;
#ifndef KOMB_FIN_PER_CU
#define KOMB_FIN_PER_CU 2
#endif
#ifndef KOMB_WIN_CAP
#define KOMB_WIN_CAP 7168
#endif
constexpr int kFinPerCu = KOMB_FIN_PER_CU;
constexpr uint32_t kWinCap = KOMB_WIN_CAP;
constexpr int kFinE = (int)(kBinEdges / kFinBlock);
constexpr int kFinU = 4;
static_assert((kWinCap * 8 + 2 * kBinEdges * 4 + 512) * kFinPerCu <= 160 * 1024, "the finishing workgroups of a CU: windows and tables are sized for gfx950's 160 KB of LDS");
static_assert(kWinCap * 8 >= (2 * kBinEdges + 4) * 4 + kBinEdges * 8, "the window buffer doubles as the table of the in-place copy");
static_assert(kFinE == 4 && kFinE <= (1 << kChunkBits), "a thread's edges are 4 consecutive ones of a chunk: their supports and own-role counts are one 16-byte vector each");
__global__ __launch_bounds__(kFinBlock, (kFinBlock / 64) * kFinPerCu / 4) void k_bin_finish(const uint32_t *__restrict__ key, const int2 *__restrict__ val,
                                                         const uint32_t *__restrict__ boff, BinGeom g,
                                                         const uint32_t *__restrict__ own, const uint32_t *__restrict__ cnt,
                                                         const uint32_t *__restrict__ bin_base,
                                                         const int2 *__restrict__ own_dense, const unsigned long long *__restrict__ ownoff,
                                                         int2 *__restrict__ dense, int64_t m,
                                                         uint2 *__restrict__ off2, int32_t *__restrict__ sup, int32_t *__restrict__ stamp, uint8_t *__restrict__ st8,
                                                         uint32_t *__restrict__ init, int32_t *__restrict__ light0)
{
    __shared__ uint32_t sh_off[kBinEdges + 4];
    __shared__ uint32_t sh_cur[kBinEdges];
    __shared__ uint32_t sh_wsum[kFinBlock / kWave];
    __shared__ int2 sh_win[kWinCap];
    __shared__ uint32_t sh_hsum[kFinBlock / kWave];
    __shared__ uint32_t sh_qbase;
    const int lane = lane_id(), w = (int)(threadIdx.x >> 6);
    uint32_t zeros = 0;
    const int32_t L1 = (int32_t)init[1];
    const bool queue_first = light0 != nullptr && L1 <= kLight;
    for (uint32_t b = blockIdx.x; b < g.nb; b += gridDim.x) {
        const uint64_t r0 = boff[b], r1 = boff[b + 1];
        const uint32_t base = bin_base[b];
        const uint32_t i0 = threadIdx.x * (uint32_t)kFinE;
        const uint64_t e0 = g.edge_of(b, i0);
        const uint32_t nin = e0 >= (uint64_t)m ? 0u : (uint32_t)min((uint64_t)kFinE, (uint64_t)m - e0);
        uint32_t c[kFinE], ow[kFinE];
        unsigned long long oo[kFinE];
        if (nin == (uint32_t)kFinE) {
            const uint4 v = *reinterpret_cast<const uint4 *>(cnt + e0);
            const uint4 q = *reinterpret_cast<const uint4 *>(own + e0);
            c[0] = v.x; c[1] = v.y; c[2] = v.z; c[3] = v.w;
            ow[0] = q.x; ow[1] = q.y; ow[2] = q.z; ow[3] = q.w;
        } else {
#pragma unroll
            for (int u = 0; u < kFinE; ++u) { const bool in = (uint32_t)u < nin; c[u] = in ? cnt[e0 + u] : 0u; ow[u] = in ? own[e0 + u] : 0u; }
        }
#pragma unroll
        for (int u = 0; u < kFinE; ++u) oo[u] = ow[u] ? ownoff[e0 + u] : 0ull;
        const uint32_t mine = c[0] + c[1] + c[2] + c[3];
        const uint32_t incl = wave_incl_scan(mine);
        uint32_t hits = 0;
#pragma unroll
        for (int u = 0; u < kFinE; ++u) hits += (queue_first && (int32_t)c[u] == L1) ? 1u : 0u;
        const uint32_t hincl = wave_incl_scan(hits);
        if (lane == kWave - 1) { sh_wsum[w] = incl; sh_hsum[w] = hincl; }
        __syncthreads();
        uint32_t before = 0, hbefore = 0, hall = 0;
#pragma unroll
        for (int i = 0; i < kFinBlock / kWave; ++i) { before += i < w ? sh_wsum[i] : 0u; hbefore += i < w ? sh_hsum[i] : 0u; hall += sh_hsum[i]; }
        if (threadIdx.x == 0 && hall) sh_qbase = atomicAdd(&init[2], hall);
        uint32_t o[kFinE + 1];
        o[0] = before + incl - mine;
#pragma unroll
        for (int u = 0; u < kFinE; ++u) o[u + 1] = o[u] + c[u];
#pragma unroll
        for (int u = 0; u < kFinE; ++u) { sh_off[i0 + u] = o[u]; sh_cur[i0 + u] = o[u]; }
        if (threadIdx.x == kFinBlock - 1) sh_off[kBinEdges] = o[kFinE];
        if (nin == (uint32_t)kFinE) {
            reinterpret_cast<uint4 *>(off2 + e0)[0] = make_uint4(base + o[0], c[0], base + o[1], c[1]);
            reinterpret_cast<uint4 *>(off2 + e0)[1] = make_uint4(base + o[2], c[2], base + o[3], c[3]);
            int4 sv, mv;
            int32_t *svp = &sv.x, *mvp = &mv.x;
#pragma unroll
            for (int u = 0; u < kFinE; ++u) {
                const bool first = queue_first && (int32_t)c[u] == L1;
                svp[u] = (int32_t)c[u];
                mvp[u] = first ? 1 : (c[u] ? alive_marker(c[u]) : 0);
                if (!c[u]) ++zeros;
            }
            *reinterpret_cast<int4 *>(sup + e0) = sv;
            *reinterpret_cast<int4 *>(stamp + e0) = mv;
            *reinterpret_cast<uchar4 *>(st8 + e0) = make_uchar4(state_of_stamp(mv.x), state_of_stamp(mv.y), state_of_stamp(mv.z), state_of_stamp(mv.w));
        } else {
#pragma unroll
            for (int u = 0; u < kFinE; ++u) if ((uint32_t)u < nin) {
                const uint64_t e = e0 + u;
                const bool first = queue_first && (int32_t)c[u] == L1;
                off2[e] = make_uint2(base + o[u], c[u]);
                sup[e] = (int32_t)c[u];
                stamp[e] = first ? 1 : (c[u] ? alive_marker(c[u]) : 0);
                st8[e] = state_of_stamp(stamp[e]);
                if (!c[u]) ++zeros;
            }
        }
        __syncthreads();
        if (hall) {
            uint32_t q = sh_qbase + hbefore + hincl - hits;
#pragma unroll
            for (int u = 0; u < kFinE; ++u) if (queue_first && (int32_t)c[u] == L1 && (uint32_t)u < nin) light0[q++] = (int32_t)(e0 + u);
        }
        const uint32_t W = sh_off[kBinEdges];
        const bool inwin = W <= kWinCap;
        for (uint64_t r = r0 + threadIdx.x; r < r1; r += (uint64_t)kFinBlock * kFinU) {
            uint32_t k[kFinU];
            int2 v[kFinU];
#pragma unroll
            for (int u = 0; u < kFinU; ++u) {
                const uint64_t rr = r + (uint64_t)u * kFinBlock;
                if (rr < r1) { k[u] = key[rr]; v[u] = val[rr]; }
            }
#pragma unroll
            for (int u = 0; u < kFinU; ++u) {
                const uint64_t rr = r + (uint64_t)u * kFinBlock;
                if (rr < r1 && (int64_t)k[u] < m) {
                    const uint32_t p = atomicAdd(&sh_cur[g.local_of(k[u])], 1u);
                    if (inwin) sh_win[p] = v[u]; else dense[base + p] = v[u];
                }
            }
        }
        if (inwin) {
            uint32_t most = 0;
#pragma unroll
            for (int u = 0; u < kFinE; ++u) most = max(most, ow[u]);
            for (uint32_t kk = 0; kk < most; ++kk) {
                int2 t[kFinE];
#pragma unroll
                for (int u = 0; u < kFinE; ++u) if (kk < ow[u]) t[u] = own_dense[oo[u] + kk];
#pragma unroll
                for (int u = 0; u < kFinE; ++u) if (kk < ow[u]) sh_win[o[u + 1] - ow[u] + kk] = t[u];
            }
        } else {
            uint32_t *tab_pre = reinterpret_cast<uint32_t *>(sh_win), *tab_dst = tab_pre + kBinEdges + 4;
            unsigned long long *tab_src = reinterpret_cast<unsigned long long *>(tab_dst + kBinEdges);
            const uint32_t mine_ow = ow[0] + ow[1] + ow[2] + ow[3];
            const uint32_t incl_ow = wave_incl_scan(mine_ow);
            __syncthreads();
            if (lane == kWave - 1) sh_wsum[w] = incl_ow;
            __syncthreads();
            uint32_t before_ow = 0, total_ow = 0;
#pragma unroll
            for (int i = 0; i < kFinBlock / kWave; ++i) { before_ow += i < w ? sh_wsum[i] : 0u; total_ow += sh_wsum[i]; }
            uint32_t run = before_ow + incl_ow - mine_ow;
#pragma unroll
            for (int u = 0; u < kFinE; ++u) {
                tab_pre[i0 + u] = run; tab_dst[i0 + u] = o[u + 1] - ow[u]; tab_src[i0 + u] = oo[u];
                run += ow[u];
            }
            if (threadIdx.x == kFinBlock - 1) tab_pre[kBinEdges] = run;
            __syncthreads();
            for (uint32_t x = threadIdx.x; x < total_ow; x += kFinBlock) {
                uint32_t lo = 0;
#pragma unroll
                for (uint32_t st = kBinEdges / 2; st > 0; st >>= 1) lo += (tab_pre[lo + st] <= x) ? st : 0u;
                const uint32_t kk = x - tab_pre[lo];
                dense[base + tab_dst[lo] + kk] = own_dense[tab_src[lo] + kk];
            }
        }
        __syncthreads();
        if (inwin) for (uint32_t j = threadIdx.x; j < W; j += kFinBlock) dense[base + j] = sh_win[j];
        __syncthreads();
    }
    block_add_min(zeros, 0x7FFFFFFF, &init[0], (int32_t *)&init[1]);
}

__global__ __launch_bounds__(kBlock) void k_peel_init(int64_t m, const uint32_t *__restrict__ off, uint2 *__restrict__ off2,
                                                      int32_t *__restrict__ sup, int32_t *__restrict__ stamp, uint8_t *__restrict__ st8,
                                                      uint32_t *__restrict__ init)
{
    uint32_t zeros = 0;
    int32_t lmin = 0x7FFFFFFF;
    for (int64_t e = (int64_t)blockIdx.x * kBlock + threadIdx.x; e < m; e += (int64_t)gridDim.x * kBlock) {
        const uint32_t b0 = off[e];
        const int32_t s0 = (int32_t)(off[e + 1] - b0);
        off2[e] = make_uint2(b0, (uint32_t)s0);
        sup[e] = s0;
        if (s0 == 0) { stamp[e] = 0; st8[e] = (uint8_t)ST_GONE; ++zeros; }
        else { const int32_t a = alive_marker((uint32_t)s0); stamp[e] = a; st8[e] = state_of_stamp(a); lmin = min(lmin, s0); }
    }
    block_add_min(zeros, lmin, &init[0], (int32_t *)&init[1]);
}

}

}
```

Baseline: 4.114 billion.

## Fuse bin count and finish into single-pass index build with atomic window claims

Replaces the separate k_bin_count kernel, the exclusive scan over bin totals, and k_bin_finish with one k_bin_build kernel. Each bin counts its records in shared memory and claims its output window with a global atomic cursor. The incidence buffer is sized from an upper bound (records claimed plus own-role entries), and a count-first fallback pass runs only when that bound is too large. Host syncs are also cut: event timing is deferred, and the moment counters and initial peel control are read back together in one staged copy. In exchange, the bin order in the incidence array is no longer deterministic, the over-allocated index uses more memory, and overflow detection now depends on a device flag.

```diff
diff --git a/komb_amd/api.py b/komb_amd/api.py
--- a/komb_amd/api.py
+++ b/komb_amd/api.py
@@ -25,7 +25,7 @@
 
 
 FORWARD_ENV_OPTIONS = False
-OPTION_NAMES = ("FINISH", "LOCAL_LIMIT", "LOCAL_ITEMS", "LOCAL_DENSITY", "LOCAL_DEFER_CHUNKS", "TAIL", "CORE_TAIL", "INDEX",
+OPTION_NAMES = ("FINISH", "LOCAL_LIMIT", "LOCAL_ITEMS", "LOCAL_DENSITY", "LOCAL_DEFER_CHUNKS", "TAIL", "CORE_TAIL", "INDEX", "INDEX_COUNT_FIRST",
                 "REC_CAP", "OWN_DENSE_CAP", "NO_OWN_DENSE", "NO_REC_SCRATCH", "NO_FIRST_QUEUE", "FULL_CAPS", "PREP_ROW_STAGE", "RETIRE_EVERY", "SHARD_ENGINE",
                 "TRI_DEBUG", "POOL_DEBUG", "BUILD_DEBUG", "LOCAL_DEBUG", "TAIL_DEBUG", "COMP_SAMPLE", "COMM_SHORT", "COMM_HEAVY", "POISON")
 
diff --git a/komb_amd/csrc/common.h b/komb_amd/csrc/common.h
--- a/komb_amd/csrc/common.h
+++ b/komb_amd/csrc/common.h
@@ -108,6 +108,33 @@
     ~EventSet() { for (hipEvent_t e : v) if (e) (void)hipEventDestroy(e); }
 };
 
+struct SpanTimers {
+    struct Span { hipEvent_t a, b; double *dst; };
+    EventSet evs;
+    std::vector<Span> spans;
+    hipError_t begin(hipStream_t s, double *dst)
+    {
+        Span p{nullptr, nullptr, dst};
+        hipError_t e = evs.make(&p.a);
+        if (e == hipSuccess) e = evs.make(&p.b);
+        if (e == hipSuccess) e = hipEventRecord(p.a, s);
+        if (e == hipSuccess) spans.push_back(p);
+        return e;
+    }
+    hipError_t end(hipStream_t s) { return spans.empty() ? hipErrorInvalidValue : hipEventRecord(spans.back().b, s); }
+    hipError_t resolve()
+    {
+        for (const Span &p : spans) {
+            float ms = 0.f;
+            const hipError_t e = hipEventElapsedTime(&ms, p.a, p.b);
+            if (e != hipSuccess) return e;
+            *p.dst += (double)ms;
+        }
+        spans.clear();
+        return hipSuccess;
+    }
+};
+
 }
 
 struct Poison {
@@ -370,6 +397,20 @@
     }
     hipError_t e = hipMemcpyAsync(dst, src, bytes, hipMemcpyDeviceToHost, ctx->stream);
     return e == hipSuccess ? hipStreamSynchronize(ctx->stream) : e;
+}
+inline hipError_t d2h_pair(komb_ctx *ctx, void *dst0, const void *src0, size_t bytes0, void *dst1, const void *src1, size_t bytes1)
+{
+    const size_t at1 = (bytes0 + 63) & ~(size_t)63;
+    if (!ctx->h_stage || at1 + bytes1 > kStageBytes) {
+        const hipError_t e = d2h(ctx, dst0, src0, bytes0);
+        return e == hipSuccess ? d2h(ctx, dst1, src1, bytes1) : e;
+    }
+    char *h = (char *)ctx->h_stage;
+    hipError_t e = hipMemcpyAsync(h, src0, bytes0, hipMemcpyDeviceToHost, ctx->stream);
+    if (e == hipSuccess) e = hipMemcpyAsync(h + at1, src1, bytes1, hipMemcpyDeviceToHost, ctx->stream);
+    if (e == hipSuccess) e = hipStreamSynchronize(ctx->stream);
+    if (e == hipSuccess) { memcpy(dst0, h, bytes0); memcpy(dst1, h + at1, bytes1); }
+    return e;
 }
 
 namespace komb {
@@ -420,7 +461,7 @@
 int peel_grid(int64_t units);
 
 template <typename F>
-int drive_peel(komb_ctx *ctx, PeelCtrl *d_ctrl, int64_t units, F &&launch, int *launches_out)
+int drive_peel(komb_ctx *ctx, PeelCtrl *d_ctrl, int64_t units, F &&launch, int *launches_out, const PeelCtrl *state_now = nullptr)
 {
 #ifndef KOMB_PEEL_BATCH
 #define KOMB_PEEL_BATCH 24
@@ -430,7 +471,8 @@
 #endif
     constexpr int kBatch = KOMB_PEEL_BATCH, kBatchShort = KOMB_PEEL_BATCH_SHORT, kShortBatches = 6;
     PeelCtrl first;
-    KOMB_HIP(ctx, d2h(ctx, &first, d_ctrl, sizeof(PeelCtrl)));
+    if (state_now) first = *state_now;
+    else KOMB_HIP(ctx, d2h(ctx, &first, d_ctrl, sizeof(PeelCtrl)));
     int32_t next = first.seq;
 #ifdef KOMB_DEBUG_SWITCHES
     if (const char *tr = getenv("KOMB_PEEL_TRACE")) {
diff --git a/komb_amd/csrc/ktruss.hip b/komb_amd/csrc/ktruss.hip
--- a/komb_amd/csrc/ktruss.hip
+++ b/komb_amd/csrc/ktruss.hip
@@ -344,7 +344,6 @@
     uint32_t *d_toff = nullptr;
     uint32_t *d_grp = nullptr;
     int32_t *d_light0 = nullptr;
-    uint32_t *d_bintot = nullptr;
     uint32_t *d_reckey = nullptr;
     int2 *d_recval = nullptr;
     const BinGeom geom = bin_geom(m);
@@ -357,6 +356,13 @@
 #endif
     st.ms_sort = 0.0; st.tri_records = 0; st.ms_compact = 0.0; st.ms_tri_count = 0.0; st.ms_tri_fill = 0.0; st.stream_retries = 0;
     st.index_layout = layout;
+    SpanTimers spans;
+    uint32_t total = 0;
+    int2 *d_inc = nullptr;
+    int32_t *d_sup = nullptr, *d_stamp = nullptr, *d_truss = nullptr;
+    uint8_t *d_st8 = nullptr;
+    bool peel_inited = false;
+    bool mom_pending = false;
     auto zero_counts = [&]() -> hipError_t { return hipMemsetAsync(d_own, 0, 2 * ((size_t)m + 1) * sizeof(uint32_t), s); };
     if (!(world == 1 && layout == IDX_STREAM)) KOMB_HIP(ctx, zero_counts());
     bool have_counts = false;
@@ -401,7 +407,7 @@
         }
         const uint32_t sentinel = geom.sentinel_base();
         uint32_t *d_key = nullptr; int2 *d_val = nullptr;
-        unsigned long long n_claimed = 0;
+        unsigned long long n_claimed = 0, own_claimed = 0;
         bool ok = false;
         st.ms_tri_fill = 0.0;
         for (int attempt = 0; attempt < 2; ++attempt) {
@@ -419,12 +425,13 @@
             if (!ok) { (void)hipGetLastError(); break; }
             KOMB_HIP(ctx, hipMemsetAsync(d_dcur, 0, 4 * sizeof(unsigned long long), s));
             const TriStream ts{d_key, d_val, d_dcur + 2, rec_cap, sentinel, geom.nb - 1u, kChunkBits};
-            ctx->timer.start(s);
+            KOMB_HIP(ctx, spans.begin(s, &st.ms_tri_fill));
             k_wedges<TRI_SINGLE><<<gws, kBlock, 0, s>>>(d_orow, d_ocol, d_line, d_wtasks, 0, n_wtasks, d_own, d_other, d_owndense, d_dcur, own_cap, d_ownoff, ts, d_scratch, ablate);
-            st.ms_tri_fill += ctx->timer.stop(s);
+            KOMB_HIP(ctx, spans.end(s));
             unsigned long long dc[4] = {0, 0, 0, 0};
             KOMB_HIP(ctx, d2h(ctx, dc, d_dcur, sizeof(dc)));
             n_claimed = dc[2];
+            own_claimed = std::min(dc[0], own_cap);
             bufs.release(d_scratch);
             if (ctx_flag(ctx, "TRI_DEBUG"))
                 fprintf(stderr, "komb triangles: stream build (attempt %d): %llu record positions claimed of %llu, dense own-role region %llu entries claimed of %llu, %llu task ranges overflowed their record buffer\n",
@@ -446,24 +453,49 @@
             uint32_t *d_key2 = nullptr; unsigned long long *d_val2 = nullptr;
             ok = bufs.alloc(&d_key2, (size_t)n_claimed + 1) == hipSuccess && bufs.alloc(&d_val2, (size_t)n_claimed + 1) == hipSuccess;
             if (ok) {
-                ctx->timer.start(s);
+                KOMB_HIP(ctx, spans.begin(s, &st.ms_sort));
                 unsigned long long *sv = nullptr;
                 if (geom.nb_bits > 0) KOMB_TRY(prim_sort_pairs_u32_u64(ctx, d_key, d_key2, (unsigned long long *)d_val, d_val2, (int64_t)n_claimed, kChunkBits, kChunkBits + geom.nb_bits, &d_skey, &sv));
                 else { d_skey = d_key; sv = (unsigned long long *)d_val; }
-                st.ms_sort = ctx->timer.stop(s);
+                KOMB_HIP(ctx, spans.end(s));
                 d_recval = (int2 *)sv;
                 if (d_skey == d_key) { bufs.release(d_key2); bufs.release(d_val2); } else { bufs.release(d_key); bufs.release(d_val); }
                 d_reckey = d_skey;
                 KOMB_HIP(ctx, bufs.alloc(&d_toff, (size_t)n_bins + 2));
-                KOMB_HIP(ctx, bufs.alloc(&d_bintot, (size_t)n_bins + 2));
                 KOMB_HIP(ctx, bufs.alloc(&d_grp, (size_t)kInitOff + 4));
                 if (!whole_peel_finish && !shard_peel_on && !ctx_flag(ctx, "NO_FIRST_QUEUE")) KOMB_HIP(ctx, bufs.alloc(&d_light0, (size_t)m));
-                ctx->timer.start(s);
-                peel_ctrl_pre(s, d_grp);
-                KOMB_HIP(ctx, hipMemsetAsync(d_mom + 5, 0, sizeof(unsigned long long), s));
+                KOMB_HIP(ctx, bufs.alloc(&d_sup, (size_t)m));
+                KOMB_HIP(ctx, bufs.alloc(&d_stamp, (size_t)m));
+                KOMB_HIP(ctx, bufs.alloc(&d_st8, (size_t)m + 16));
+                KOMB_HIP(ctx, bufs.alloc(&d_truss, (size_t)m));
+                auto bin_build = [&](unsigned long long cap) -> hipError_t {
+                    peel_ctrl_pre(s, d_grp);
+                    hipError_t e = hipMemsetAsync(d_mom + 5, 0, 2 * sizeof(unsigned long long), s);
+                    if (e != hipSuccess) return e;
+                    k_bin_build<<<grid_for(n_bins, 1, 256 * kFinPerCu), kFinBlock, 0, s>>>(d_reckey, d_recval, d_toff, geom, d_own, d_owndense, d_ownoff, d_inc, cap,
+                                                                                 d_mom + 5, d_mom + 6, m, d_cnt_ref ? d_cnt : nullptr,
+                                                                                 d_off2, d_sup, d_stamp, d_st8, d_grp + kInitOff, d_light0);
+                    return hipGetLastError();
+                };
+                unsigned long long inc_cap = n_claimed + own_claimed;
+                KOMB_HIP(ctx, spans.begin(s, &st.ms_compact));
                 k_bin_offsets<<<grid_for(n_bins + 1), kBlock, 0, s>>>(d_skey, (int64_t)n_claimed, geom, d_toff);
-                k_bin_count<<<grid_for(n_bins, 1, 256 * 8), kBlock, 0, s>>>(d_skey, d_toff, geom, d_own, m, d_cnt, d_bintot, d_mom + 5, (int32_t *)(d_grp + kInitOff + 1));
-                st.ms_compact = ctx->timer.stop(s);
+                if (inc_cap > 0xFFFFFFF0ull || ctx_flag(ctx, "INDEX_COUNT_FIRST")) {
+                    KOMB_HIP(ctx, bin_build(0ull));
+                    unsigned long long sum = 0;
+                    KOMB_HIP(ctx, d2h(ctx, &sum, d_mom + 5, sizeof(sum)));
+                    st.triangles = (int64_t)(sum / 3);
+                    if (sum > 0xFFFFFFF0ull)
+                        KOMB_FAIL(ctx, KOMB_ERR_LIMIT, "graph has %llu triangles; the incidence index is limited to 2^32-16 entries (3 per triangle)", sum / 3);
+                    inc_cap = sum;
+                }
+                total = (uint32_t)inc_cap;
+                KOMB_HIP(ctx, bufs.alloc(&d_inc, (size_t)inc_cap));
+                KOMB_HIP(ctx, bin_build(inc_cap));
+                KOMB_HIP(ctx, spans.end(s));
+                peel_inited = true; mom_pending = true;
+                bufs.release(d_toff); bufs.release((void *)d_recval); bufs.release(d_reckey);
+                bufs.release(d_owndense); bufs.release(d_ownoff); bufs.release(d_dcur);
                 st.tri_records = (int64_t)n_claimed;
             } else (void)hipGetLastError();
         }
@@ -473,7 +505,8 @@
             d_owndense = nullptr; d_ownoff = nullptr; d_dcur = nullptr;
             KOMB_HIP(ctx, zero_counts());
             KOMB_HIP(ctx, hipMemsetAsync(d_mom + 5, 0, sizeof(unsigned long long), s));
-            st.ms_tri_fill = 0.0;
+            st.ms_tri_fill = 0.0; st.ms_sort = 0.0;
+            spans.spans.clear();
             layout = IDX_TWO_PASS;
         }
     }
@@ -493,40 +526,25 @@
         }
     }
     st.index_layout = layout;
-    {
-        unsigned long long mom[9];
-        KOMB_HIP(ctx, d2h(ctx, mom, d_mom, sizeof(mom)));
+    auto check_mom = [&](const unsigned long long *mom) -> int {
         st.triangles = (int64_t)(mom[5] / 3);
-        bufs.release(d_mom);
         if (mom[8] != 0)
             KOMB_FAIL(ctx, KOMB_ERR_DEVICE, "komb_truss_run_sharded: %llu edges whose all-reduced support differs from the support of the index build", mom[8]);
         if (mom[5] > 0xFFFFFFF0ull)
             KOMB_FAIL(ctx, KOMB_ERR_LIMIT, "graph has %llu triangles; the incidence index is limited to 2^32-16 entries (3 per triangle)",
                       mom[5] / 3);
-    }
-    bufs.release(d_cnt_ref);
-    uint32_t total = 0;
-    const uint32_t sum_supports = (uint32_t)st.triangles * 3u;
-    int2 *d_inc = nullptr;
-    int32_t *d_sup = nullptr, *d_stamp = nullptr, *d_truss = nullptr;
-    uint8_t *d_st8 = nullptr;
-    bool peel_inited = false;
-    if (layout == IDX_STREAM) {
-        KOMB_TRY(prim_exclusive_sum_u32(ctx, d_bintot, d_bintot, n_bins + 1));
-        total = sum_supports;
-        KOMB_HIP(ctx, bufs.alloc(&d_inc, (size_t)total));
-        KOMB_HIP(ctx, bufs.alloc(&d_sup, (size_t)m));
-        KOMB_HIP(ctx, bufs.alloc(&d_stamp, (size_t)m));
-        KOMB_HIP(ctx, bufs.alloc(&d_st8, (size_t)m + 16));
-        KOMB_HIP(ctx, bufs.alloc(&d_truss, (size_t)m));
-        ctx->timer.start(s);
-        k_bin_finish<<<grid_for(n_bins, 1, 256 * kFinPerCu), kFinBlock, 0, s>>>(d_reckey, d_recval, d_toff, geom, d_own, d_cnt, d_bintot, d_owndense, d_ownoff, d_inc, m,
-                                                                      d_off2, d_sup, d_stamp, d_st8, d_grp + kInitOff, d_light0);
-        st.ms_compact += ctx->timer.stop(s);
-        peel_inited = true;
-        bufs.release(d_toff); bufs.release(d_bintot); bufs.release((void *)d_recval); bufs.release(d_reckey);
-        bufs.release(d_owndense); bufs.release(d_ownoff); bufs.release(d_dcur);
-    } else {
+        if (mom_pending && mom[6] != 0)
+            KOMB_FAIL(ctx, KOMB_ERR_DEVICE, "k-truss index build: %llu entries do not fit the %u the enumeration's claims allow for", mom[5], total);
+        return KOMB_OK;
+    };
+    if (!mom_pending) {
+        unsigned long long mom[9];
+        KOMB_HIP(ctx, d2h(ctx, mom, d_mom, sizeof(mom)));
+        KOMB_TRY(check_mom(mom));
+        bufs.release(d_mom);
+    }
+    if (layout == IDX_TWO_PASS) {
+        bufs.release(d_cnt_ref); d_cnt_ref = nullptr;
         KOMB_HIP(ctx, bufs.alloc(&d_off, (size_t)m + 1));
         KOMB_TRY(prim_exclusive_sum_u32(ctx, d_cnt, d_off, m + 1));
         KOMB_HIP(ctx, d2h(ctx, &total, d_off + m, sizeof(uint32_t)));
@@ -536,9 +554,9 @@
         k_back_cursors<<<ge, kBlock, 0, s>>>(d_off, m, d_other);
         k_triangles<TRI_SINGLE><<<gt, kBlock, 0, s>>>(d_orow, d_ocol, nv, 0, ntasks, d_own, d_other, d_off, d_inc, ablate, tri_tv);
         st.ms_tri_fill = ctx->timer.stop(s);
-    }
-    st.ms_support = st.ms_tri_count + st.ms_tri_fill + st.ms_sort + st.ms_compact;
-    bufs.release(d_cnt); bufs.release(d_own);
+        st.ms_support = st.ms_tri_count + st.ms_tri_fill + st.ms_sort + st.ms_compact;
+    }
+    bufs.release(d_cnt_ref); bufs.release(d_cnt); bufs.release(d_own);
 
     phase.next("truss: peel");
     PeelCtrl *d_ctrl = nullptr;
@@ -658,6 +676,17 @@
         k_peel_init<<<grid_for(m, kBlock, 1024), kBlock, 0, s>>>(m, d_off, d_off2, d_sup, d_stamp, d_st8, d_grp + kInitOff);
     }
     peel_ctrl_init(s, d_ctrl, d_grp, (uint32_t)m, tail_limit);
+    PeelCtrl ctrl0;
+    bool have_ctrl0 = false;
+    if (mom_pending) {
+        unsigned long long mom[9];
+        KOMB_HIP(ctx, d2h_pair(ctx, &ctrl0, d_ctrl, sizeof(PeelCtrl), mom, d_mom, sizeof(mom)));
+        have_ctrl0 = true;
+        bufs.release(d_mom);
+        KOMB_HIP(ctx, spans.resolve());
+        st.ms_support = st.ms_tri_count + st.ms_tri_fill + st.ms_sort + st.ms_compact;
+        KOMB_TRY(check_mom(mom));
+    }
     int launches = 0, rc = KOMB_OK;
     st.truss_tail_runs = 0; st.ms_tail = 0.0;
     st.truss_local_units = 0; st.truss_local_sweeps = 0; st.truss_local_items = 0; st.ms_truss_local = 0.0;
@@ -677,7 +706,8 @@
         fc.done = rc == KOMB_OK ? 1 : 2; fc.n_levels = ss.levels; fc.n_rounds = ss.rounds; fc.n_scans = ss.scans; fc.max_level = ss.max_level;
         ctx->h_ctrl[0] = fc;
     } else if (whole_peel_finish) {
-        rc = d2h(ctx, &ctx->h_ctrl[0], d_ctrl, sizeof(PeelCtrl)) == hipSuccess ? KOMB_OK : KOMB_ERR_DEVICE;
+        if (have_ctrl0) ctx->h_ctrl[0] = ctrl0;
+        else rc = d2h(ctx, &ctx->h_ctrl[0], d_ctrl, sizeof(PeelCtrl)) == hipSuccess ? KOMB_OK : KOMB_ERR_DEVICE;
         if (rc == KOMB_OK && !ctx->h_ctrl[0].done) rc = (fin == FIN_LOCAL) ? run_local() : run_tail(nullptr, (uint32_t)m);
     } else {
         ctx->h_ctrl[0].done = 0;
@@ -692,7 +722,7 @@
         int batch = 0;
         rc = drive_peel(ctx, d_ctrl, m, [&](int32_t launch) {
             k_peel_step<TrussProblem><<<gp, kPeelBlock, 0, s>>>(d_ctrl, d_grp, Q, P, launch);
-        }, &batch);
+        }, &batch, have_ctrl0 && guard == 0 && !whole_peel_finish && !shard_peel_on ? &ctrl0 : nullptr);
         launches += batch;
     }
     st.ms_peel = ctx->timer.stop(s);
diff --git a/komb_amd/csrc/truss_index.h b/komb_amd/csrc/truss_index.h
--- a/komb_amd/csrc/truss_index.h
+++ b/komb_amd/csrc/truss_index.h
@@ -51,50 +51,6 @@
     block_add_u64(t, bad);
 }
 
-__global__ __launch_bounds__(kBlock) void k_bin_count(const uint32_t *__restrict__ key, const uint32_t *__restrict__ boff, BinGeom g,
-                                                      const uint32_t *__restrict__ own, int64_t m, uint32_t *__restrict__ sum,
-                                                      uint32_t *__restrict__ bin_total, unsigned long long *__restrict__ total,
-                                                      int32_t *__restrict__ min_pos)
-{
-    __shared__ uint32_t sh_cnt[kBinEdges];
-    __shared__ uint32_t sh_part[kBlock / kWave];
-    unsigned long long t = 0;
-    int32_t lmin = 0x7FFFFFFF;
-    for (uint32_t b = blockIdx.x; b < g.nb; b += gridDim.x) {
-        for (uint32_t i = threadIdx.x; i < kBinEdges; i += kBlock) sh_cnt[i] = 0u;
-        __syncthreads();
-        const uint32_t r0 = boff[b], r1 = boff[b + 1];
-        for (uint32_t r = r0 + threadIdx.x; r < r1; r += kBlock) {
-            const uint32_t k = key[r];
-            if ((int64_t)k < m) atomicAdd(&sh_cnt[g.local_of(k)], 1u);
-        }
-        __syncthreads();
-        uint32_t tb = 0;
-        for (uint32_t i = threadIdx.x; i < kBinEdges; i += kBlock) {
-            const uint64_t e = g.edge_of(b, i);
-            if (e >= (uint64_t)m) continue;
-            const uint32_t c = own[e] + sh_cnt[i];
-            sum[e] = c;
-            tb += c;
-            if (c) lmin = min(lmin, (int32_t)c);
-        }
-        tb = wave_sum(tb);
-        if (lane_id() == 0) sh_part[threadIdx.x >> 6] = tb;
-        __syncthreads();
-        if (threadIdx.x == 0) {
-            uint32_t all = 0;
-            for (int i = 0; i < kBlock / kWave; ++i) all += sh_part[i];
-            bin_total[b] = all;
-            t += all;
-        }
-        __syncthreads();
-    }
-    if (blockIdx.x == 0 && threadIdx.x == 0) { sum[m] = 0u; bin_total[g.nb] = 0u; }
-    if (threadIdx.x == 0 && t) atomicAdd(total, t);
-    lmin = wave_min(lmin);
-    if (lane_id() == 0 && lmin != 0x7FFFFFFF) atomicMin(min_pos, lmin);
-}
-
 constexpr int kFinBlock = 512;
 #ifndef KOMB_FIN_PER_CU
 #define KOMB_FIN_PER_CU 2
@@ -106,115 +62,141 @@
 constexpr uint32_t kWinCap = KOMB_WIN_CAP;
 constexpr int kFinE = (int)(kBinEdges / kFinBlock);
 constexpr int kFinU = 4;
-static_assert((kWinCap * 8 + 2 * kBinEdges * 4 + 512) * kFinPerCu <= 160 * 1024, "the finishing workgroups of a CU: windows and tables are sized for gfx950's 160 KB of LDS");
+static_assert((kWinCap * 8 + kBinEdges * 4 + 512) * kFinPerCu <= 160 * 1024, "the finishing workgroups of a CU: windows and tables are sized for gfx950's 160 KB of LDS");
 static_assert(kWinCap * 8 >= (2 * kBinEdges + 4) * 4 + kBinEdges * 8, "the window buffer doubles as the table of the in-place copy");
 static_assert(kFinE == 4 && kFinE <= (1 << kChunkBits), "a thread's edges are 4 consecutive ones of a chunk: their supports and own-role counts are one 16-byte vector each");
-__global__ __launch_bounds__(kFinBlock, (kFinBlock / 64) * kFinPerCu / 4) void k_bin_finish(const uint32_t *__restrict__ key, const int2 *__restrict__ val,
-                                                         const uint32_t *__restrict__ boff, BinGeom g,
-                                                         const uint32_t *__restrict__ own, const uint32_t *__restrict__ cnt,
-                                                         const uint32_t *__restrict__ bin_base,
+__global__ __launch_bounds__(kFinBlock, (kFinBlock / 64) * kFinPerCu / 4) void k_bin_build(const uint32_t *__restrict__ key, const int2 *__restrict__ val,
+                                                         const uint32_t *__restrict__ boff, BinGeom g, const uint32_t *__restrict__ own,
                                                          const int2 *__restrict__ own_dense, const unsigned long long *__restrict__ ownoff,
-                                                         int2 *__restrict__ dense, int64_t m,
+                                                         int2 *__restrict__ dense, unsigned long long dense_cap,
+                                                         unsigned long long *__restrict__ window_cursor, unsigned long long *__restrict__ overflow,
+                                                         int64_t m, uint32_t *__restrict__ cnt_out,
                                                          uint2 *__restrict__ off2, int32_t *__restrict__ sup, int32_t *__restrict__ stamp, uint8_t *__restrict__ st8,
                                                          uint32_t *__restrict__ init, int32_t *__restrict__ light0)
 {
-    __shared__ uint32_t sh_off[kBinEdges + 4];
     __shared__ uint32_t sh_cur[kBinEdges];
     __shared__ uint32_t sh_wsum[kFinBlock / kWave];
     __shared__ int2 sh_win[kWinCap];
     __shared__ uint32_t sh_hsum[kFinBlock / kWave];
     __shared__ uint32_t sh_qbase;
+    __shared__ unsigned long long sh_base;
     const int lane = lane_id(), w = (int)(threadIdx.x >> 6);
+    const uint32_t i0 = threadIdx.x * (uint32_t)kFinE;
     uint32_t zeros = 0;
-    const int32_t L1 = (int32_t)init[1];
-    const bool queue_first = light0 != nullptr && L1 <= kLight;
+    int32_t lmin = 0x7FFFFFFF;
+    const bool queue_first = light0 != nullptr;
+    static_assert(kLight >= 1, "the first frontier (support 1) must be light units");
+#pragma unroll
+    for (int u = 0; u < kFinE; ++u) sh_cur[i0 + u] = 0u;
+    if (blockIdx.x == 0 && threadIdx.x == 0 && cnt_out) cnt_out[m] = 0u;
+    __syncthreads();
     for (uint32_t b = blockIdx.x; b < g.nb; b += gridDim.x) {
         const uint64_t r0 = boff[b], r1 = boff[b + 1];
-        const uint32_t base = bin_base[b];
-        const uint32_t i0 = threadIdx.x * (uint32_t)kFinE;
         const uint64_t e0 = g.edge_of(b, i0);
         const uint32_t nin = e0 >= (uint64_t)m ? 0u : (uint32_t)min((uint64_t)kFinE, (uint64_t)m - e0);
         uint32_t c[kFinE], ow[kFinE];
         unsigned long long oo[kFinE];
         if (nin == (uint32_t)kFinE) {
-            const uint4 v = *reinterpret_cast<const uint4 *>(cnt + e0);
             const uint4 q = *reinterpret_cast<const uint4 *>(own + e0);
-            c[0] = v.x; c[1] = v.y; c[2] = v.z; c[3] = v.w;
             ow[0] = q.x; ow[1] = q.y; ow[2] = q.z; ow[3] = q.w;
         } else {
 #pragma unroll
-            for (int u = 0; u < kFinE; ++u) { const bool in = (uint32_t)u < nin; c[u] = in ? cnt[e0 + u] : 0u; ow[u] = in ? own[e0 + u] : 0u; }
+            for (int u = 0; u < kFinE; ++u) ow[u] = (uint32_t)u < nin ? own[e0 + u] : 0u;
+        }
+        uint32_t k[kFinU];
+        int2 v[kFinU];
+#pragma unroll
+        for (int u = 0; u < kFinU; ++u) {
+            const uint64_t rr = r0 + threadIdx.x + (uint64_t)u * kFinBlock;
+            k[u] = 0xFFFFFFFFu;
+            if (rr < r1) { k[u] = key[rr]; v[u] = val[rr]; }
+        }
+#pragma unroll
+        for (int u = 0; u < kFinU; ++u) if ((int64_t)k[u] < m) atomicAdd(&sh_cur[g.local_of(k[u])], 1u);
+        for (uint64_t r = r0 + threadIdx.x + (uint64_t)kFinBlock * kFinU; r < r1; r += kFinBlock) {
+            const uint32_t kk = key[r];
+            if ((int64_t)kk < m) atomicAdd(&sh_cur[g.local_of(kk)], 1u);
         }
 #pragma unroll
         for (int u = 0; u < kFinE; ++u) oo[u] = ow[u] ? ownoff[e0 + u] : 0ull;
+        __syncthreads();
+#pragma unroll
+        for (int u = 0; u < kFinE; ++u) c[u] = ow[u] + sh_cur[i0 + u];
         const uint32_t mine = c[0] + c[1] + c[2] + c[3];
         const uint32_t incl = wave_incl_scan(mine);
         uint32_t hits = 0;
 #pragma unroll
-        for (int u = 0; u < kFinE; ++u) hits += (queue_first && (int32_t)c[u] == L1) ? 1u : 0u;
+        for (int u = 0; u < kFinE; ++u) hits += (queue_first && c[u] == 1u) ? 1u : 0u;
         const uint32_t hincl = wave_incl_scan(hits);
         if (lane == kWave - 1) { sh_wsum[w] = incl; sh_hsum[w] = hincl; }
         __syncthreads();
-        uint32_t before = 0, hbefore = 0, hall = 0;
-#pragma unroll
-        for (int i = 0; i < kFinBlock / kWave; ++i) { before += i < w ? sh_wsum[i] : 0u; hbefore += i < w ? sh_hsum[i] : 0u; hall += sh_hsum[i]; }
-        if (threadIdx.x == 0 && hall) sh_qbase = atomicAdd(&init[2], hall);
+        uint32_t before = 0, hbefore = 0, hall = 0, W = 0;
+#pragma unroll
+        for (int i = 0; i < kFinBlock / kWave; ++i) { before += i < w ? sh_wsum[i] : 0u; W += sh_wsum[i]; hbefore += i < w ? sh_hsum[i] : 0u; hall += sh_hsum[i]; }
+        const bool inwin = W <= kWinCap;
+        unsigned long long claimed = 0ull;
+        uint32_t qclaimed = 0u;
+        if (threadIdx.x == 0) {
+            if (W) claimed = atomicAdd(window_cursor, (unsigned long long)W);
+            if (hall) qclaimed = atomicAdd(&init[2], hall);
+        }
         uint32_t o[kFinE + 1];
         o[0] = before + incl - mine;
 #pragma unroll
         for (int u = 0; u < kFinE; ++u) o[u + 1] = o[u] + c[u];
 #pragma unroll
-        for (int u = 0; u < kFinE; ++u) { sh_off[i0 + u] = o[u]; sh_cur[i0 + u] = o[u]; }
-        if (threadIdx.x == kFinBlock - 1) sh_off[kBinEdges] = o[kFinE];
+        for (int u = 0; u < kFinE; ++u) sh_cur[i0 + u] = o[u];
         if (nin == (uint32_t)kFinE) {
-            reinterpret_cast<uint4 *>(off2 + e0)[0] = make_uint4(base + o[0], c[0], base + o[1], c[1]);
-            reinterpret_cast<uint4 *>(off2 + e0)[1] = make_uint4(base + o[2], c[2], base + o[3], c[3]);
             int4 sv, mv;
             int32_t *svp = &sv.x, *mvp = &mv.x;
 #pragma unroll
             for (int u = 0; u < kFinE; ++u) {
-                const bool first = queue_first && (int32_t)c[u] == L1;
+                const bool first = queue_first && c[u] == 1u;
                 svp[u] = (int32_t)c[u];
                 mvp[u] = first ? 1 : (c[u] ? alive_marker(c[u]) : 0);
-                if (!c[u]) ++zeros;
+                if (!c[u]) ++zeros; else lmin = min(lmin, (int32_t)c[u]);
             }
             *reinterpret_cast<int4 *>(sup + e0) = sv;
             *reinterpret_cast<int4 *>(stamp + e0) = mv;
             *reinterpret_cast<uchar4 *>(st8 + e0) = make_uchar4(state_of_stamp(mv.x), state_of_stamp(mv.y), state_of_stamp(mv.z), state_of_stamp(mv.w));
+            if (cnt_out) *reinterpret_cast<uint4 *>(cnt_out + e0) = make_uint4(c[0], c[1], c[2], c[3]);
         } else {
 #pragma unroll
             for (int u = 0; u < kFinE; ++u) if ((uint32_t)u < nin) {
                 const uint64_t e = e0 + u;
-                const bool first = queue_first && (int32_t)c[u] == L1;
-                off2[e] = make_uint2(base + o[u], c[u]);
+                const bool first = queue_first && c[u] == 1u;
+                const int32_t mk = first ? 1 : (c[u] ? alive_marker(c[u]) : 0);
                 sup[e] = (int32_t)c[u];
-                stamp[e] = first ? 1 : (c[u] ? alive_marker(c[u]) : 0);
-                st8[e] = state_of_stamp(stamp[e]);
-                if (!c[u]) ++zeros;
-            }
-        }
-        __syncthreads();
-        if (hall) {
-            uint32_t q = sh_qbase + hbefore + hincl - hits;
-#pragma unroll
-            for (int u = 0; u < kFinE; ++u) if (queue_first && (int32_t)c[u] == L1 && (uint32_t)u < nin) light0[q++] = (int32_t)(e0 + u);
-        }
-        const uint32_t W = sh_off[kBinEdges];
-        const bool inwin = W <= kWinCap;
-        for (uint64_t r = r0 + threadIdx.x; r < r1; r += (uint64_t)kFinBlock * kFinU) {
-            uint32_t k[kFinU];
-            int2 v[kFinU];
+                stamp[e] = mk;
+                st8[e] = state_of_stamp(mk);
+                if (cnt_out) cnt_out[e] = c[u];
+                if (!c[u]) ++zeros; else lmin = min(lmin, (int32_t)c[u]);
+            }
+        }
+        if (!inwin && threadIdx.x == 0) { sh_base = claimed; sh_qbase = qclaimed; }
+        __syncthreads();
+        unsigned long long base = 0ull;
+        bool fits = true;
+        if (!inwin) { base = sh_base; fits = base + W <= dense_cap; }
+#pragma unroll
+        for (int u = 0; u < kFinU; ++u) {
+            if ((int64_t)k[u] < m) {
+                const uint32_t p = atomicAdd(&sh_cur[g.local_of(k[u])], 1u);
+                if (inwin) sh_win[p] = v[u]; else if (fits) dense[base + p] = v[u];
+            }
+        }
+        for (uint64_t r = r0 + threadIdx.x + (uint64_t)kFinBlock * kFinU; r < r1; r += (uint64_t)kFinBlock * kFinU) {
 #pragma unroll
             for (int u = 0; u < kFinU; ++u) {
                 const uint64_t rr = r + (uint64_t)u * kFinBlock;
+                k[u] = 0xFFFFFFFFu;
                 if (rr < r1) { k[u] = key[rr]; v[u] = val[rr]; }
             }
 #pragma unroll
             for (int u = 0; u < kFinU; ++u) {
-                const uint64_t rr = r + (uint64_t)u * kFinBlock;
-                if (rr < r1 && (int64_t)k[u] < m) {
+                if ((int64_t)k[u] < m) {
                     const uint32_t p = atomicAdd(&sh_cur[g.local_of(k[u])], 1u);
-                    if (inwin) sh_win[p] = v[u]; else dense[base + p] = v[u];
+                    if (inwin) sh_win[p] = v[u]; else if (fits) dense[base + p] = v[u];
                 }
             }
         }
@@ -229,6 +211,7 @@
 #pragma unroll
                 for (int u = 0; u < kFinE; ++u) if (kk < ow[u]) sh_win[o[u + 1] - ow[u] + kk] = t[u];
             }
+            if (threadIdx.x == 0) { sh_base = claimed; sh_qbase = qclaimed; }
         } else {
             uint32_t *tab_pre = reinterpret_cast<uint32_t *>(sh_win), *tab_dst = tab_pre + kBinEdges + 4;
             unsigned long long *tab_src = reinterpret_cast<unsigned long long *>(tab_dst + kBinEdges);
@@ -248,7 +231,7 @@
             }
             if (threadIdx.x == kFinBlock - 1) tab_pre[kBinEdges] = run;
             __syncthreads();
-            for (uint32_t x = threadIdx.x; x < total_ow; x += kFinBlock) {
+            if (fits) for (uint32_t x = threadIdx.x; x < total_ow; x += kFinBlock) {
                 uint32_t lo = 0;
 #pragma unroll
                 for (uint32_t st = kBinEdges / 2; st > 0; st >>= 1) lo += (tab_pre[lo + st] <= x) ? st : 0u;
@@ -257,10 +240,28 @@
             }
         }
         __syncthreads();
-        if (inwin) for (uint32_t j = threadIdx.x; j < W; j += kFinBlock) dense[base + j] = sh_win[j];
-        __syncthreads();
-    }
-    block_add_min(zeros, 0x7FFFFFFF, &init[0], (int32_t *)&init[1]);
+        base = sh_base;
+        fits = base + W <= dense_cap;
+        const uint32_t b32 = (uint32_t)base;
+        if (nin == (uint32_t)kFinE) {
+            reinterpret_cast<uint4 *>(off2 + e0)[0] = make_uint4(b32 + o[0], c[0], b32 + o[1], c[1]);
+            reinterpret_cast<uint4 *>(off2 + e0)[1] = make_uint4(b32 + o[2], c[2], b32 + o[3], c[3]);
+        } else {
+#pragma unroll
+            for (int u = 0; u < kFinE; ++u) if ((uint32_t)u < nin) off2[e0 + u] = make_uint2(b32 + o[u], c[u]);
+        }
+        if (hall) {
+            uint32_t q = sh_qbase + hbefore + hincl - hits;
+#pragma unroll
+            for (int u = 0; u < kFinE; ++u) if (queue_first && c[u] == 1u && (uint32_t)u < nin) light0[q++] = (int32_t)(e0 + u);
+        }
+        if (inwin && fits) for (uint32_t j = threadIdx.x; j < W; j += kFinBlock) dense[base + j] = sh_win[j];
+        if (!fits && threadIdx.x == 0) *overflow = 1ull;
+#pragma unroll
+        for (int u = 0; u < kFinE; ++u) sh_cur[i0 + u] = 0u;
+        __syncthreads();
+    }
+    block_add_min(zeros, lmin, &init[0], (int32_t *)&init[1]);
 }
 
 __global__ __launch_bounds__(kBlock) void k_peel_init(int64_t m, const uint32_t *__restrict__ off, uint2 *__restrict__ off2,
```

Result: faster. 4.185 billion (median of 6 runs) (+1.7%).
